# gradslam/gradslam

Measured on AMD Instinct MI355X. Metric: frames/sec PointFusion 640x480 RGB-D, higher is better.
Workload: dtype f32

## Files before the change

gradslam_amd/_C.py:

```python
import ctypes as C
import os

import torch

_HERE = os.path.dirname(os.path.abspath(__file__))
LIB_PATH = os.environ.get("GRADSLAM_HIP_LIB") or os.path.join(_HERE, "csrc", "libgradslam_hip.so")
if os.environ.get("GRADSLAM_HIP_LIB"):
    import warnings
    warnings.warn("GRADSLAM_HIP_LIB overrides the product library: %s" % LIB_PATH, RuntimeWarning)
ABI_VERSION = 3

_lib = None

_vp, _i64, _i32, _f = C.c_void_p, C.c_int64, C.c_int, C.c_float


class IcpParams(C.Structure):
    _fields_ = [("mode", C.c_int), ("numiters", C.c_int), ("damp", C.c_float),
                ("dist_thresh", C.c_float), ("lambda_max", C.c_float), ("B", C.c_float),
                ("B2", C.c_float), ("nu", C.c_float)]


class MapView(C.Structure):
    _fields_ = [("points", C.c_void_p), ("normals", C.c_void_p), ("colors", C.c_void_p), ("ccounts", C.c_void_p),
                ("capacity", C.c_int64), ("n_bound", C.c_int64), ("n_dev", C.c_void_p)]


class LocalizeSeq(C.Structure):
    _fields_ = [("vertex", C.c_void_p), ("depth", C.c_void_p), ("K16", C.c_void_p), ("prev_pose16", C.c_void_p),
                ("map", MapView), ("out_pose16", C.c_void_p), ("scratch", C.c_void_p)]


class UpdateSeq(C.Structure):
    _fields_ = [("map", MapView), ("vertex", C.c_void_p), ("normal", C.c_void_p), ("depth", C.c_void_p),
                ("rgb", C.c_void_p), ("alpha", C.c_void_p), ("pose16", C.c_void_p), ("K16", C.c_void_p),
                ("gvertex", C.c_void_p), ("gnormal", C.c_void_p), ("best_pix", C.c_void_p),
                ("new_count_out", C.c_void_p), ("scratch", C.c_void_p)]


class StepSeq(C.Structure):
    _fields_ = [("depth", C.c_void_p), ("rgb", C.c_void_p), ("K16", C.c_void_p), ("prev_pose16", C.c_void_p),
                ("out_pose16", C.c_void_p), ("vertex", C.c_void_p), ("normal", C.c_void_p), ("alpha", C.c_void_p),
                ("gvertex", C.c_void_p), ("gnormal", C.c_void_p), ("best_pix", C.c_void_p),
                ("new_count_out", C.c_void_p), ("map", MapView), ("loc_scratch", C.c_void_p),
                ("upd_scratch", C.c_void_p)]


class RenderSeq(C.Structure):
    _fields_ = [("map", MapView), ("poses16", C.c_void_p), ("K16", C.c_void_p), ("depth", C.c_void_p),
                ("color", C.c_void_p), ("normal", C.c_void_p), ("confidence", C.c_void_p), ("index", C.c_void_p),
                ("scratch", C.c_void_p)]


class RenderBackwardSeq(C.Structure):
    _fields_ = [("map", MapView), ("poses16", C.c_void_p), ("K16", C.c_void_p), ("index", C.c_void_p),
                ("depth_bar", C.c_void_p), ("color_bar", C.c_void_p), ("normal_bar", C.c_void_p),
                ("confidence_bar", C.c_void_p), ("points_bar", C.c_void_p), ("normals_bar", C.c_void_p),
                ("colors_bar", C.c_void_p), ("ccounts_bar", C.c_void_p), ("poses_bar", C.c_void_p),
                ("scratch", C.c_void_p)]


_PROTOS = {
    "gs_abi_version": [],
    "gs_last_error": [],
    "gs_scratch_bytes": [_i64, _i64],
    "gs_profile_begin": [_i32],
    "gs_profile_end": [],
    "gs_profile_read": [_i32, C.POINTER(C.c_double), C.POINTER(C.c_int64), C.POINTER(C.c_double)],
    "gs_frame_maps_f32": [_vp, _vp, _i32, _i32, _f, _vp, _vp, _vp, _vp, _vp],
    "gs_global_maps_f32": [_vp, _vp, _vp, _vp, _i32, _i32, _vp, _vp, _vp],
    "gs_alpha_f32": [_vp, _i64, _f, _f, _vp, _vp],
    "gs_alpha_backward_f32": [_vp, _i64, _f, _f, _vp, _vp, _vp, _vp],
    "gs_downsample_frame_f32": [_vp, _vp, _vp, _vp, _i32, _i32, _i32, _vp, _vp, _vp, _vp, _vp, _vp],
    "gs_project_map_f32": [_vp, _i64, _vp, _vp, _i32, _i32, _vp, _vp],
    "gs_active_table_i64": [_vp, _i64, _i32, _i64, _vp, _vp, _vp, _vp],
    "gs_select_targets_f32": [_vp, _i64, _i32, _i32, _vp, _vp, _vp, _vp, _vp, _vp, _i64, _vp, _vp, _vp],
    "gs_downsample_table_f32": [_vp, _i64, _i32, _vp, _vp, _vp, _vp, _vp, _vp, _vp, _vp, _vp],
    "gs_knn1_f32": [_vp, _i64, _vp, _i64, _vp, _vp, _vp, _vp],
    "gs_knn1_grid_scratch_bytes": [_i64, _i64],
    "gs_knn1_grid_f32": [_vp, _i64, _vp, _i64, _vp, _vp, _vp, C.POINTER(C.c_int64), _vp],
    "gs_gauss_newton_rows_f32": [_vp, _i64, _vp, _vp, _i64, _f, _vp, _vp, _vp, _vp, _vp, _vp],
    "gs_solve_normal_eq_f32": [_vp, _vp, _vp, _i64, _i32, _f, _vp, _vp],
    "gs_se3_exp_f32": [_vp, _vp, _vp],
    "gs_se3_exp_backward_f32": [_vp, _vp, _vp, _vp],
    "gs_transform_points_f32": [_vp, _i64, _vp, _vp, _vp],
    "gs_icp_scratch_bytes": [_i64, _i64],
    "gs_icp_f32": [_vp, _i64, _vp, _vp, _i64, _vp, _vp, C.POINTER(IcpParams), _vp, _vp, _vp, _vp],
    "gs_icp_trace_f32": [_vp, _i32, _vp, _vp],
    "gs_icp_dc_f32": [_vp, _i64, _vp, _vp, _vp, _i64, _vp, _vp, _vp, C.POINTER(IcpParams), _vp, _vp, _vp, _vp],
    "gs_frame_maps_backward_f32": [_vp, _vp, _i32, _i32, _f, _vp, _vp, _vp, _vp, _vp, _vp, _vp, _vp],
    "gs_frame_maps_backward_kbar_scratch_bytes": [_i32, _i32],
    "gs_global_maps_backward_f32": [_vp, _vp, _vp, _vp, _i32, _i32, _vp, _vp, _vp],
    "gs_downsample_frame_backward_f32": [_vp, _vp, _i32, _i32, _i32, _vp, _vp, _vp],
    "gs_icp_tape_bytes": [_i64, _i32],
    "gs_icp_tape_f32": [_vp, _i64, _vp, _vp, _i64, _vp, _vp, C.POINTER(IcpParams), _vp, _vp, _vp, _vp, _vp],
    "gs_icp_backward_scratch_bytes": [_i64, _i64],
    "gs_icp_backward_f32": [_vp, _vp, _i64, _vp, _vp, _i64, _vp, C.POINTER(IcpParams), _vp, _vp, _vp, _vp, _vp, _vp,
                            _vp],
    "gs_similar_rows_f32": [_vp, _i64, _vp, _vp, _vp, _vp, _i32, _f, _f, _vp, _vp],
    "gs_best_unique_rows_f32": [_vp, _i64, _vp, _vp, _vp, _i32, _i32, _i64, _vp, _vp, _vp, _vp, _vp],
    "gs_associate_f32": [_vp, _i64, _vp, _vp, _vp, _vp, _vp, _i32, _i32, _f, _f, _vp, _vp, _vp, _vp],
    "gs_best_table_i64": [_vp, _i32, _i32, _i64, _vp, _vp, _vp, _vp],
    "gs_rows_to_best_pix": [_vp, _i64, _i32, _i32, _vp, _vp],
    "gs_fuse_append_f32": [_vp, _vp, _vp, _vp, _i64, _i64, _vp, _vp, _vp, _vp, _vp, _vp, _i32, _i32, _i32,
                           _vp, _vp, _vp],
    "gs_append_valid_f32": [_vp, _vp, _vp, _vp, _i64, _i64, _vp, _vp, _vp, _vp, _vp, _i32, _i32, _vp, _vp, _vp],
    "gs_ingest_depth_u16_f32": [_vp, _i32, _i32, _vp, _i32, _i32, C.c_double, _vp],
    "gs_ingest_color_u8_f32": [_vp, _i32, _i32, _vp, _i32, _i32, _i32, _vp],
    "gs_ingest_frames_native_f32": [_vp, _vp, _i64, _i32, _i32, C.c_double, _i32, _vp, _vp, _vp],
    "gs_host_device_pointer": [_vp, C.POINTER(C.c_void_p)],
    "gs_global_maps_pose_backward_scratch_bytes": [_i32, _i32],
    "gs_global_maps_pose_backward_f32": [_vp, _vp, _vp, _vp, _vp, _i32, _i32, _vp, _vp, _vp],
    "gs_fuse_append_backward_f32": [_vp, _vp, _vp, _vp, _i64, _vp, _vp, _vp, _vp, _vp, _vp, _i32, _i32, _i32, _vp, _vp,
                                    _vp, _vp, _i64, _vp, _vp, _vp, _vp, _vp, _vp, _vp, _vp, _vp, _vp],
    "gs_update_map_scratch_bytes": [_i64, _i32, _i32],
    "gs_update_map_fusion_dc_f32": [_vp, _vp, _vp, _vp, _i64, _vp, _i64, _vp, _vp, _vp, _vp, _vp, _vp, _vp, _i32, _i32,
                                    _f, _f, _i32, _vp, _vp, _vp, _vp, _vp, _vp],
    "gs_icp_map_dc_f32": [_vp, _i64, _vp, _vp, _vp, _vp, _i64, _vp, _i32, _i32, _vp, _vp, C.POINTER(IcpParams), _vp, _vp,
                          _vp],
    "gs_lattice_source_f32": [_vp, _vp, _vp, _i32, _i32, _i32, _vp, _vp],
    "gs_relative_pose_f32": [_vp, _vp, _i64, _vp, _vp],
    "gs_project_map_dc_f32": [_vp, _i64, _vp, _vp, _vp, _i32, _i32, _vp, _vp],
    "gs_select_targets_dc_f32": [_vp, _i64, _vp, _i32, _i32, _vp, _vp, _vp, _vp, _vp, _vp, _i64, _vp, _vp, _vp],
    "gs_associate_dc_f32": [_vp, _i64, _vp, _vp, _vp, _vp, _vp, _vp, _i32, _i32, _f, _f, _vp, _vp, _vp, _vp],
    "gs_fuse_append_dc_f32": [_vp, _vp, _vp, _vp, _i64, _vp, _i64, _vp, _vp, _vp, _vp, _vp, _vp, _i32, _i32, _i32,
                              _vp, _vp, _vp],
    "gs_append_valid_dc_f32": [_vp, _vp, _vp, _vp, _i64, _vp, _i64, _vp, _vp, _vp, _vp, _vp, _i32, _i32, _vp, _vp,
                               _vp],
    "gs_frame_maps_batch_f32": [_vp, _i64, _i64, _vp, _i32, _i32, _i32, _i32, _f, _vp, _vp, _vp, _vp],
    "gs_localize_scratch_bytes": [_i32, _i32, _i32, _i64],
    "gs_localize_batch_f32": [C.POINTER(LocalizeSeq), _i32, _i32, _i32, _i32, C.POINTER(IcpParams), _vp],
    "gs_update_map_fusion_batch_f32": [C.POINTER(UpdateSeq), _i32, _i32, _i32, _f, _f, _i32, _vp],
    "gs_project_points_f32": [_vp, _i32, _i64, _vp, _i64, _vp, _vp],
    "gs_unproject_points_f32": [_vp, _i32, _i64, _vp, _i64, _vp, _vp, _vp],
    "gs_lie_small_f32": [_i32, _vp, _vp, _vp],
    "gs_localize_far_stats_i64": [_vp, _i32, _i32, _i32, _i64, C.POINTER(C.c_int64), _vp],
    "gs_localize_list_stats_i64": [_vp, _i32, _i32, _i32, _i64, C.POINTER(C.c_int64), _vp],
    "gs_localize_solve_stats_i64": [_vp, _i32, _i32, _i32, _i64, C.POINTER(C.c_int64), _vp],
    "gs_pointfusion_step_batch_f32": [C.POINTER(StepSeq), _i32, _i32, _i32, _i32, C.POINTER(IcpParams), _f, _f, _f, _i32, _vp],
    "gs_render_scratch_bytes": [_i32, _i32, _i32],
    "gs_render_map_dc_f32": [C.POINTER(RenderSeq), _i32, _i32, _i32, _i32, _i32, _f, _i32, _vp],
    "gs_render_backward_scratch_bytes": [_i32, _i32, _i32, _i64],
    "gs_render_map_backward_dc_f32": [C.POINTER(RenderBackwardSeq), _i32, _i32, _i32, _i32, _i32, _vp],
}
_RESTYPE = {"gs_last_error": C.c_char_p, "gs_scratch_bytes": _i64, "gs_icp_scratch_bytes": _i64,
            "gs_knn1_grid_scratch_bytes": _i64, "gs_update_map_scratch_bytes": _i64, "gs_global_maps_pose_backward_scratch_bytes": _i64, "gs_icp_tape_bytes": _i64, "gs_icp_backward_scratch_bytes": _i64,
            "gs_localize_scratch_bytes": _i64, "gs_frame_maps_backward_kbar_scratch_bytes": _i64,
            "gs_render_scratch_bytes": _i64, "gs_render_backward_scratch_bytes": _i64}
EXPORTS = tuple(_PROTOS)


class HipExtensionError(RuntimeError):
    pass


def lib():
    global _lib
    if _lib is None:
        if not os.path.exists(LIB_PATH):
            raise HipExtensionError(
                "gradslam_amd: %s is missing. Build it with `python -m gradslam_amd.csrc.build` "
                "(hipcc --offload-arch=gfx950). There is no CPU / PyTorch fallback." % LIB_PATH)
        handle = C.CDLL(LIB_PATH)
        for name, argtypes in _PROTOS.items():
            fn = getattr(handle, name)
            fn.argtypes = argtypes
            fn.restype = _RESTYPE.get(name, C.c_int)
        if handle.gs_abi_version() != ABI_VERSION:
            raise HipExtensionError("libgradslam_hip.so ABI %d != expected %d; rebuild"
                                    % (handle.gs_abi_version(), ABI_VERSION))
        _lib = handle
    return _lib


def check(status, what):
    if status != 0:
        raise HipExtensionError("%s failed (code %d): %s" % (what, status, lib().gs_last_error().decode()))


def require_device(*tensors):
    dev = None
    for t in tensors:
        if t is None:
            continue
        if not t.is_cuda:
            raise HipExtensionError(
                "gradslam_amd kernels run on the GPU only (got a %s tensor). Move the data to a HIP "
                "device; there is no CPU fallback." % t.device)
        if not t.is_contiguous():
            raise HipExtensionError("internal error: non-contiguous tensor passed to the HIP library")
        if dev is None:
            dev = t.device
        elif t.device != dev:
            raise HipExtensionError("tensors live on different devices: %s vs %s" % (dev, t.device))
    return dev


def ptr(t):
    return None if t is None else C.c_void_p(t.data_ptr())


def stream(device):
    return C.c_void_p(torch.cuda.current_stream(device).cuda_stream)


class Workspace:
    _instances = {}

    def __init__(self, device):
        self.device = device
        self._bufs = {}

    @classmethod
    def get(cls, device):
        device = torch.device(device)
        if device.index is None:
            device = torch.device("cuda", torch.cuda.current_device())
        key = (device, torch.cuda.current_stream(device).cuda_stream)
        ws = cls._instances.get(key)
        if ws is None:
            ws = cls._instances[key] = Workspace(device)
        return ws

    def bytes(self, name, nbytes):
        buf = self._bufs.get(name)
        if buf is None or buf.numel() < nbytes:
            nbytes = int(nbytes * 1.5) + 4096
            buf = self._bufs[name] = torch.empty(nbytes, dtype=torch.uint8, device=self.device)
        return buf

    def scratch(self, n_map, n_pix):
        return self.bytes("scratch", lib().gs_scratch_bytes(int(n_map), int(n_pix)))

    def tensor(self, name, shape, dtype):
        n = 1
        for s in shape:
            n *= int(s)
        item = torch.empty((), dtype=dtype).element_size()
        buf = self.bytes(name, max(n, 1) * item)
        return buf[: n * item].view(dtype).view(*shape)
```

gradslam_amd/csrc/gs_icp_loop.hip:

```cpp
#include <stdlib.h>
#include <string.h>

#include <memory>
#include <mutex>
#include <type_traits>

#include "gs_env.h"
#include "gs_icp_math.h"
#include "gs_knn.h"
#include "gs_knn_bbox.h"

constexpr int GS_ICP_MAX_ITERS = 1024;
struct GsIcpState {
  IcpSmall s[2];
  float trace[GS_ICP_MAX_ITERS * 12];
};

struct TapePtrs {
  float* src;
  int32_t* idx;
  float* sys;
};
GS_DEV void tape_write_sys(float* __restrict__ sys, int it, const double* S, float damp) {
  float* t = sys + 28 * it;
// ... 1127 lines not shown
  float* lattice;
  GsIcpState* state;
  float* out_pose16;
  char* clear_ptr;
  int64_t* n_valid;
  int* far_n;
  int* lstat;
  float4* wl_cq;
  unsigned* sync;
};
struct LocBatch {
  int B, W, ds, Wl;
  int64_t n_lat;
  size_t clear_bytes;
  float damp;
  int numiters;
  int count_valid;
  LocSeq s[GS_MAX_BATCH];
};
constexpr int LP_CLEAR_ITEMS = 8;

GS_DEV void loc_prep_block(const LocBatch& lb, const unsigned bid, const unsigned nb_lat) {
  const LocSeq& q = lb.s[bid % lb.B];
  const unsigned blk = bid / lb.B;
  if (blk < nb_lat) {
    const int64_t e = (int64_t)blk * 256 + threadIdx.x;
    int valid = 0;
    if (e < lb.n_lat) {
      const int64_t p = (e / lb.Wl) * lb.ds * (int64_t)lb.W + (e % lb.Wl) * lb.ds;
      float g0 = __builtin_nanf(""), g1 = g0, g2 = g0;
      if (q.depth[p] > 0.0f) {
        float T[12];
#pragma unroll
        for (int i = 0; i < 12; ++i) T[i] = q.pose16[i];
        gs_rigid_fma(T, q.vertex[3 * p], q.vertex[3 * p + 1], q.vertex[3 * p + 2], g0, g1, g2);
        valid = 1;
      }
      q.lattice[3 * e] = g0; q.lattice[3 * e + 1] = g1; q.lattice[3 * e + 2] = g2;
      if (q.wl_cq) q.wl_cq[e] = make_float4(0.0f, 0.0f, 0.0f, 0.0f);
    }
    const unsigned long long m = lb.count_valid ? __ballot(valid) : 0ull;
    if ((threadIdx.x & 63) == 0 && m) atomicAdd(reinterpret_cast<unsigned long long*>(q.n_valid), (unsigned long long)__popcll(m));
    if (blk == 0 && threadIdx.x == 0) {
      IcpSmall sm;
      for (int i = 0; i < 16; ++i) {
        const float id = (i % 5 == 0) ? 1.0f : 0.0f;
        sm.T_total[i] = id; sm.T_step[i] = id; sm.Tr[i] = id;
      }
      for (int i = 0; i < 8; ++i) sm.xi[i] = 0.0f;
      sm.damp = lb.damp;
      sm.err = 0.0f;
      sm.pad[0] = sm.pad[1] = 0.0f;
      q.state->s[0] = sm;
      q.state->s[1] = sm;
      if (q.far_n)
        for (int i = 0; i < FS_FAR_PASSES; ++i) q.far_n[i] = 0;
      if (q.lstat)
        for (int i = 0; i < 3 * GL_STAT_LAUNCHES; ++i) q.lstat[i] = 0;
      if (q.sync)
        for (int i = 0; i < PS_WORDS; ++i) q.sync[i] = 0u;
      if (lb.numiters == 0) icp_write_result(sm, q.pose16, q.out_pose16);
    }
    return;
  }
  float4* dst = reinterpret_cast<float4*>(q.clear_ptr);
  const size_t n16 = lb.clear_bytes / 16;
  const size_t base = (size_t)(blk - nb_lat) * 256 * LP_CLEAR_ITEMS + threadIdx.x;
#pragma unroll
  for (int u = 0; u < LP_CLEAR_ITEMS; ++u) {
    const size_t i = base + (size_t)u * 256;
    if (i < n16) dst[i] = make_float4(0.0f, 0.0f, 0.0f, 0.0f);
  }
}
__global__ void __launch_bounds__(256) gs_loc_prep_kernel(const LocBatch lb, unsigned nb_lat) {
  loc_prep_block(lb, blockIdx.x, nb_lat);
}
static_assert(GB_BLOCK == 256, "lattice and bbox blocks share a launch");
__global__ void __launch_bounds__(256) gs_loc_prep_bbox_kernel(const LocBatch lb, const GsGridBatch gb, const unsigned nb_lat,
                                                               const float u_hi, const float v_hi) {
  const unsigned n_prep = (unsigned)lb.B * nb_lat;
  if (blockIdx.x < n_prep) loc_prep_block(lb, blockIdx.x, nb_lat);
  else gridb_bbox_block(gb, blockIdx.x - n_prep, u_hi, v_hi);
}

struct IcpRowsBatch {
  int B;
  const double* in[GS_MAX_BATCH];
  double* out[GS_MAX_BATCH];
};
__global__ void __launch_bounds__(FS_BLOCK) gs_icp_reduce_rows_batch_kernel(const IcpRowsBatch rb, GsCount n_src_c) {
  __shared__ double S[32];
  __shared__ double sub[FS_BLOCK / 32][32];
  const int nrows = (int)((gs_count(n_src_c) + FS_QPB - 1) / FS_QPB);
  icp_sum_rows<FS_BLOCK>(rb.in[blockIdx.x], nrows, S, sub);
  if (threadIdx.x < LIN_NV) rb.out[blockIdx.x][threadIdx.x] = S[threadIdx.x];
}

struct IcpFinishBatch {
  int B;
  const double* partials_in[GS_MAX_BATCH];
  GsIcpState* st[GS_MAX_BATCH];
  const float* compose16[GS_MAX_BATCH];
  float* out_T16[GS_MAX_BATCH];
  unsigned* sync[GS_MAX_BATCH];
  int nb, h0;
};
__global__ void __launch_bounds__(FS_BLOCK) gs_icp_finish_batch_kernel(const IcpFinishBatch fb, GsCount n_src_c, int buf,
                                                                       gs_icp_params prm) {
  __shared__ double red[FS_BLOCK / GS_WAVE];
  const int b = blockIdx.x;
  const int nrows_in = (int)((gs_count(n_src_c) + FS_QPB - 1) / FS_QPB);
  const double e1 = icp_sum_col27<FS_BLOCK>(fb.partials_in[b], nrows_in, red);
  if (threadIdx.x != 0) return;
  GsIcpState* st = fb.st[b];
  IcpSmall sm = st->s[buf];
  const int it = prm.numiters - 1;
  icp_update_math((float)e1, sm, prm, it < GS_ICP_MAX_ITERS ? st->trace + 12 * it : nullptr);
  st->s[buf ^ 1] = sm;
  icp_write_result(sm, fb.compose16[b], fb.out_T16[b]);
  if (unsigned* sy = fb.sync[b]) {
    const unsigned arrived = sy[PS_ARRIVED], want = (unsigned)fb.nb * (unsigned)(2 * prm.numiters - fb.h0);
    if (!(sy[PS_ERROR] == 0u && arrived == want && sy[PS_TICKET] >= (unsigned)fb.nb))
      for (int i = 0; i < 16; ++i) fb.out_T16[b][i] = __builtin_nanf("");
    sy[PS_NB] = (unsigned)fb.nb;
    sy[PS_H0] = (unsigned)fb.h0;
  }
}

static int64_t loc_lattice(int H, int W, int ds) { return (int64_t)((H + ds - 1) / ds) * ((W + ds - 1) / ds); }

struct ListMem {
  float4* lq;
  uint32_t* ls;
  int* stat;
};

struct FarMem {
  uint32_t* c;
  float4* cq;
  int* idx;
  int* n;
};

struct FarBuildSeq {
  const float* src;
  const int* idx;
  const int* n;
  const GsGrid* gp;
  const int* cell_start;
  const float4* sorted;
  float* d2prev;
  FarMem m;
};
struct FarBuildBatch {
  int B;
  FarBuildSeq s[GS_MAX_BATCH];
};
constexpr int FAR_BLOCK = 512;
constexpr int FAR_BLOCKS_PER_SEQ = 64;
__global__ void __launch_bounds__(FAR_BLOCK) gs_icp_far_build_kernel(const FarBuildBatch fb) {
  const FarBuildSeq& q = fb.s[blockIdx.x % fb.B];
  const int blk = (int)(blockIdx.x / fb.B);
  const int n = *q.n;
  if (blk >= n) return;
  constexpr int NG = FAR_BLOCK / FS_HG;
  __shared__ float qs[NG][3];
  __shared__ float d1_s[NG];
  __shared__ uint8_t flag_s[NG];
  __shared__ int unres_q[NG], sq_s[NG];
  __shared__ int unres_n;
  __shared__ uint32_t stage_s[NG][GS_FAR_SLOTS + 4];
  const GsGrid g = *q.gp;
  const int grp = threadIdx.x / FS_HG, l16 = threadIdx.x & (FS_HG - 1);
  for (int base = blk; base < n; base += FAR_BLOCKS_PER_SEQ * NG) {
    if (threadIdx.x == 0) unres_n = 0;
    __syncthreads();
    const int e = base + grp * FAR_BLOCKS_PER_SEQ;
    if (e < n) {
      const int sq = q.idx[e];
      const float hx = q.src[3 * (int64_t)sq], hy = q.src[3 * (int64_t)sq + 1], hz = q.src[3 * (int64_t)sq + 2];
      const float4 found = q.m.cq[sq];
      const float d1 = sqrtf(found.x);
      const int kdone = (int)found.y;
      if (kdone >= 0) {
        const float R = far_emit_cube<FS_HG>(g, q.cell_start, q.sorted, hx, hy, hz, l16, d1, kdone, stage_s[grp],
                                             reinterpret_cast<int*>(&stage_s[grp][GS_FAR_SLOTS]));
        for (int u = l16; u < GS_FAR_SLOTS; u += FS_HG) q.m.c[GS_FAR_SLOTS * (int64_t)sq + u] = stage_s[grp][u];
        if (l16 == 0) {
          q.m.cq[sq] = make_float4(hx, hy, hz, R);
          if (R > 0.0f) q.d2prev[sq] = __uint_as_float(__float_as_uint(q.d2prev[sq]) | 0x80000000u);
        }
      } else if (l16 == 0) {
        qs[grp][0] = hx; qs[grp][1] = hy; qs[grp][2] = hz;
        d1_s[grp] = d1;
        sq_s[grp] = sq;
        unres_q[atomicAdd(&unres_n, 1)] = grp;
      }
    }
    __syncthreads();
    const int nun = unres_n;
    for (int u = 0; u < nun; u += FS_BQ) {
      const int nq = nun - u < FS_BQ ? nun - u : FS_BQ;
      block_brute_collect_multi<FAR_BLOCK, FS_BQ>(qs, unres_q + u, nq, q.sorted, q.cell_start[g.ncell], d1_s,
                                                  GS_FAR_RADD * g.c, sq_s, q.m.cq, q.m.c, flag_s);
      if ((int)threadIdx.x < nq) {
        const int gq = unres_q[u + threadIdx.x];
        const int s2 = sq_s[gq];
        if (flag_s[gq]) q.d2prev[s2] = __uint_as_float(__float_as_uint(q.d2prev[s2]) | 0x80000000u);
      }
    }
    __syncthreads();
  }
}

static int64_t loc_rows(const gs_map_view& m) { return m.capacity > m.n_bound ? m.capacity : m.n_bound; }

struct LocLayout {
  int64_t n_lat, rows;
  IcpLayout sc;
  size_t lattice, pix, n_valid, icp, lq, ls, lstat, far_c, far_cq, far_idx, far_n, far_out4, total;
};
static LocLayout loc_layout(int64_t n_lat, int64_t rows) {
  GsTake take;
  LocLayout L;
  L.n_lat = n_lat; L.rows = rows > 0 ? rows : 1;
  L.lattice = take(gs_align(12 * (size_t)n_lat));
  L.pix = take(gs_align(4 * (size_t)L.rows));
  L.n_valid = take(256);
  L.sc = icp_layout(n_lat, L.rows);
  L.icp = take(L.sc.total);
  L.lq = take(gs_align(16 * (size_t)n_lat));
  L.ls = take(gs_align(4 * GL_SLOTS * (size_t)n_lat));
  L.lstat = take(gs_align(4 * 3 * GL_STAT_LAUNCHES));
  L.far_c = take(gs_align(4 * GS_FAR_SLOTS * (size_t)n_lat));
  L.far_cq = take(gs_align(16 * (size_t)n_lat));
  L.far_idx = take(gs_align(4 * FS_FAR_PASSES * (size_t)n_lat));
  L.far_n = take(256);
  L.far_out4 = L.far_n + 4 * 8;
  static_assert(FS_FAR_PASSES <= 8, "the far-list counters run into the result words");
  L.total = take.end;
  return L;
}
static bool loc_lists_fit(const LocLayout& L) { return L.total - (L.icp + L.sc.partials[1]) >= sizeof(double) * LIN_NV * FS_BLOCK; }

extern "C" int64_t gs_localize_scratch_bytes(int H, int W, int ds, int64_t n_map_bound) {
  if (H < 1 || W < 1 || ds < 1) return 0;
  return (int64_t)loc_layout(loc_lattice(H, W, ds), n_map_bound).total;
}

struct LocCarve {
  float* lattice; int32_t* pix; int64_t* n_valid;
  IcpScratch sc; GridMem gm; ListMem lm;
  FarMem fm; int* far_out4;
};
static LocCarve loc_carve(void* p, const LocLayout& L) {
  const IcpScratch sc = icp_carve(gs_at<char>(p, L.icp), L.sc);
  return LocCarve{gs_at<float>(p, L.lattice), gs_at<int32_t>(p, L.pix), gs_at<int64_t>(p, L.n_valid), sc,
                  grid_carve(sc.grid, L.n_lat, L.rows),
                  ListMem{gs_at<float4>(p, L.lq), gs_at<uint32_t>(p, L.ls), gs_at<int>(p, L.lstat)},
                  FarMem{gs_at<uint32_t>(p, L.far_c), gs_at<float4>(p, L.far_cq), gs_at<int>(p, L.far_idx), gs_at<int>(p, L.far_n)},
                  gs_at<int>(p, L.far_out4)};
}
static LocCarve loc_carve_of(const void* scratch, int H, int W, int ds, int64_t map_rows) {
  return loc_carve(const_cast<void*>(scratch), loc_layout(loc_lattice(H, W, ds), map_rows));
}

struct IcpEnginePlan {
  bool far_on, wide_on, lists_on, persist_on;
  bool binned_normals;
  bool reduce_rows;
  int lists_from;
  IcpHalfPlan half;
  int ps_it0, ps_nb, ps_upb;
  float weak_room;
  int lmode(int it, bool look_ahead) const {
    if (!lists_on || it < lists_from) return 0;
    if (it > lists_from) return 2;
    return look_ahead ? (persist_on ? 3 : 1) : 0;
  }
};
static IcpEnginePlan icp_engine_plan(const GsEnv& env, const IcpDevice& dev, int B, int64_t n_lat, int numiters,
                                     const LocLayout* layouts) {
  IcpEnginePlan p;
  const int64_t rows = (int64_t)icp_rows(n_lat);
  p.binned_normals = env.icp_binned_normals; p.weak_room = env.icp_weak_room;
  p.lists_from = env.icp_lists_from >= 0 ? env.icp_lists_from : FS_LISTS_FROM;
  p.reduce_rows = rows > FS_REDUCE_ROWS;
  p.far_on = env.icp_far && numiters > 0;
  p.wide_on = env.icp_wide && !p.far_on && numiters > 0;
  p.ps_upb = (int)gs_ceil_div(rows, PS_CUS_PER_XCD);
  p.ps_nb = (int)gs_ceil_div(rows, p.ps_upb > 0 ? p.ps_upb : 1);
  const bool persist_asked = env.icp_persist && env.icp_lists && !p.far_on && B <= (int)GS_XCDS && p.ps_upb <= PS_UPB &&
                             numiters > p.lists_from + 1 && !env.icp_timeline && !env.icp_lanes_set && dev.ps_fits &&
                             p.binned_normals;
  p.half = icp_half_plan(env, dev.cus, n_lat, B, p.far_on ? 4 : (persist_asked ? 2 : 8));
  p.lists_on = env.icp_lists && !p.far_on && p.half.upb * p.half.G * FS_QPB <= FS_BLOCK;
  for (int b = 0; b < B && p.lists_on; ++b) p.lists_on = loc_lists_fit(layouts[b]);
  p.persist_on = persist_asked && p.half.G == 2 && p.lists_on;
  p.ps_it0 = p.persist_on ? p.lists_from + 1 : numiters;
  return p;
}

static void loc_bind(const gs_localize_seq* seqs, int B, int H, int W, int ds, const gs_icp_params* prm,
                     const IcpEnginePlan& plan, LocCarve* c, LocBatch& lb, GsGridBatch& gb) {
  lb.B = gb.B = B; lb.W = gb.W = W; gb.H = H; lb.ds = gb.ds = ds;
  lb.Wl = (W + ds - 1) / ds; lb.n_lat = loc_lattice(H, W, ds); lb.damp = prm->damp; lb.numiters = prm->numiters;
  gb.cells_cap = gs_knn_grid_cells_cap(lb.n_lat);
  for (int b = 0; b < B; ++b) {
    const gs_localize_seq& q = seqs[b];
    if (!plan.binned_normals) c[b].gm.sorted_n = nullptr;
    lb.s[b] = LocSeq{q.vertex, q.depth, q.prev_pose16, c[b].lattice, c[b].sc.state, q.out_pose16,
                     reinterpret_cast<char*>(c[b].gm.g), c[b].n_valid, c[b].fm.n, c[b].lm.stat,
                     plan.wide_on ? c[b].fm.cq : nullptr, c[b].sc.sync};
    gb.s[b] = GsGridSeq{q.map.points, GsCount{q.map.n_bound, q.map.n_dev}, c[b].pix, q.prev_pose16, q.K16,
                        plan.binned_normals ? q.map.normals : nullptr, c[b].gm};
  }
  lb.count_valid = g_gs_prof_on ? 1 : 0;
  lb.clear_bytes = gs_knn_grid_clear_bytes(c[0].gm, gb.cells_cap);
}

static int loc_prep(const gs_localize_seq* seqs, const LocBatch& lb, const GsGridBatch& gb, hipStream_t st, bool grid_cleared) {
  const int B = lb.B;
  if (g_gs_prof_on)
    for (int b = 0; b < B; ++b) GS_HIP(hipMemsetAsync(lb.s[b].n_valid, 0, 8, st));
  const unsigned nb_lat = (unsigned)gs_ceil_div(lb.n_lat, 256);
  const unsigned nb_clear = (unsigned)gs_ceil_div((int64_t)(lb.clear_bytes / 16), 256 * LP_CLEAR_ITEMS);
  double bytes = 0.0;
  for (int b = 0; b < B; ++b) bytes += 28.0 * lb.n_lat + 24.0 * seqs[b].map.n_bound + 16.0 * gb.cells_cap;
  GsProf prof(GS_PROF_COMPACT, bytes, st, grid_cleared ? 4 : 5);
  if (grid_cleared) {
    const float u_hi = (float)((double)gb.W - 0.999), v_hi = (float)((double)gb.H - 0.999);
    hipLaunchKernelGGL(gs_loc_prep_bbox_kernel, dim3((unsigned)B * nb_lat + gs_knn_gridb_bbox_blocks(gb)), dim3(256), 0, st,
                       lb, gb, nb_lat, u_hi, v_hi);
    return gs_knn_grid_build_batch(gb, st, true);
  }
  hipLaunchKernelGGL(gs_loc_prep_kernel, dim3((unsigned)B * (nb_lat + nb_clear)), dim3(256), 0, st, lb, nb_lat);
  return gs_knn_grid_build_batch(gb, st);
}

static int loc_prof_bytes(int B, const LocCarve* c, int64_t n_lat, int numiters, hipStream_t st, double* bytes) {
  for (int b = 0; b < B; ++b) {
    unsigned hits = 0; int64_t nv = 0;
    GS_HIP(hipMemcpyAsync(&hits, c[b].gm.bbox + 6, 4, hipMemcpyDeviceToHost, st));
    GS_HIP(hipMemcpyAsync(&nv, c[b].n_valid, 8, hipMemcpyDeviceToHost, st));
    GS_HIP(hipStreamSynchronize(st));
    *bytes += icp_alg_bytes(numiters, n_lat, nv, hits);
  }
  return GS_OK;
}

static void loc_half_iterations(const gs_localize_seq* seqs, int B, const IcpEnginePlan& plan, const LocCarve* c,
                                int64_t n_lat, const gs_icp_params* prm, hipStream_t st) {
  const GsCount n_src_c{n_lat, nullptr};
  const FarMem no_far{nullptr, nullptr, nullptr, nullptr};
  IcpHalfBatch hb;
  hb.B = B; hb.weak_room = plan.weak_room;
  for (int it = 0; it < plan.ps_it0; ++it) {
    int h = 2 * it;
    for (int b = 0; b < B; ++b) {
      const gs_localize_seq& q = seqs[b];
      const IcpScratch& sc = c[b].sc; const GridMem& gm = c[b].gm;
      const FarMem& fm = plan.far_on ? c[b].fm : no_far;
      const float* cur_in = it == 0 ? c[b].lattice : (((it - 1) & 1) ? sc.srcB : sc.srcA);
      float* cur = (it & 1) ? sc.srcB : sc.srcA;
      hb.s[b] = IcpHalfSeq{cur_in, cur, q.map.points, q.map.normals, GsCount{q.map.n_bound, q.map.n_dev}, gm.g,
                           gm.cell_start, gm.sorted, gm.sorted_n, reinterpret_cast<float*>(sc.best),
                           sc.partials[(h + 1) & 1], sc.partials[h & 1], &sc.state->s[h & 1], &sc.state->s[(h + 1) & 1],
                           sc.state->trace, nullptr, nullptr, nullptr, fm.cq, fm.c, fm.idx, fm.n};
      hb.w[b] = plan.wide_on ? IcpHalfWide{c[b].fm.cq, c[b].fm.c} : IcpHalfWide{nullptr, nullptr};
      hb.l[b] = plan.lists_on ? IcpHalfLists{c[b].lm.lq, c[b].lm.ls, c[b].lm.stat, sc.sync + PS_WEAK}
                              : IcpHalfLists{nullptr, nullptr, nullptr, nullptr};
    }
    icp_half_launch<true>(plan.half, hb, n_src_c, prm, it, 0, st, plan.lmode(it, false));
    if (plan.far_on && fs_far_pass(it) >= 0) {
      const int fp = fs_far_pass(it);
      FarBuildBatch fbb; fbb.B = B;
      for (int b = 0; b < B; ++b)
        fbb.s[b] = FarBuildSeq{(it & 1) ? c[b].sc.srcB : c[b].sc.srcA, c[b].fm.idx + (int64_t)fp * n_lat, c[b].fm.n + fp,
                               c[b].gm.g, c[b].gm.cell_start, c[b].gm.sorted, reinterpret_cast<float*>(c[b].sc.best), c[b].fm};
      hipLaunchKernelGGL(gs_icp_far_build_kernel, dim3((unsigned)B * FAR_BLOCKS_PER_SEQ), dim3(FAR_BLOCK), 0, st, fbb);
    }
    ++h;
    if (plan.reduce_rows) {
      IcpRowsBatch rb; rb.B = B;
      for (int b = 0; b < B; ++b) { rb.in[b] = c[b].sc.partials[(h + 1) & 1]; rb.out[b] = c[b].sc.rowred; }
      hipLaunchKernelGGL(gs_icp_reduce_rows_batch_kernel, dim3((unsigned)B), dim3(FS_BLOCK), 0, st, rb, n_src_c);
    }
    for (int b = 0; b < B; ++b) {
      const IcpScratch& sc = c[b].sc;
      IcpHalfSeq& u = hb.s[b];
      u.src_in = (it & 1) ? sc.srcB : sc.srcA; u.src_out = nullptr;
      u.partials_in = plan.reduce_rows ? sc.rowred : sc.partials[(h + 1) & 1];
      u.partials_out = sc.partials[h & 1];
      u.st_in = &sc.state->s[h & 1]; u.st_out = &sc.state->s[(h + 1) & 1];
    }
    icp_half_launch<false>(plan.half, hb, n_src_c, prm, it, plan.reduce_rows ? 1 : 0, st, plan.lmode(it, true));
  }
}

static void loc_persist(const gs_localize_seq* seqs, int B, const IcpEnginePlan& plan, const LocCarve* c, int64_t n_lat,
                        const gs_icp_params* prm, hipStream_t st) {
  IcpPersistBatch pb;
  pb.B = B; pb.nb = plan.ps_nb; pb.upb = plan.ps_upb; pb.h0 = 2 * plan.ps_it0; pb.tl_h = 0; pb.timeline = nullptr;
  for (int b = 0; b < B; ++b) {
    const gs_localize_seq& q = seqs[b];
    const IcpScratch& sc = c[b].sc; const GridMem& gm = c[b].gm;
    pb.s[b] = IcpPersistSeq{((plan.ps_it0 - 1) & 1) ? sc.srcB : sc.srcA, GsCount{q.map.n_bound, q.map.n_dev}, gm.g, gm.cell_start,
                            gm.sorted, gm.sorted_n, {sc.partials[0], sc.partials[1]}, sc.state, c[b].lm.lq, c[b].lm.ls,
                            c[b].lm.stat, plan.wide_on ? c[b].fm.cq : nullptr, plan.wide_on ? c[b].fm.c : nullptr, sc.sync};
  }
#ifdef GS_ICP_TIMELINE
  ps_tl_arm(pb, prm->numiters, st);
#endif
  hipLaunchKernelGGL(gs_icp_persist_kernel, dim3(GS_XCDS * PS_CUS_PER_XCD), dim3(PS_BLOCK), 0, st, pb, n_lat, prm->dist_thresh, *prm);
#ifdef GS_ICP_TIMELINE
  ps_tl_dump(pb, st);
#endif
}

static void loc_finish(const gs_localize_seq* seqs, int B, const IcpEnginePlan& plan, const LocCarve* c, int64_t n_lat,
                       const gs_icp_params* prm, hipStream_t st) {
  const int h = 2 * prm->numiters;
  GsProf prof(GS_PROF_SOLVE, 1.0, st);
  IcpFinishBatch fb;
  fb.B = B; fb.nb = plan.persist_on ? plan.ps_nb : 0; fb.h0 = plan.persist_on ? 2 * plan.ps_it0 : 0;
  for (int b = 0; b < B; ++b) {
    fb.partials_in[b] = c[b].sc.partials[(h + 1) & 1];
    fb.st[b] = c[b].sc.state; fb.compose16[b] = seqs[b].prev_pose16; fb.out_T16[b] = seqs[b].out_pose16;
    fb.sync[b] = plan.persist_on ? c[b].sc.sync : nullptr;
  }
  hipLaunchKernelGGL(gs_icp_finish_batch_kernel, dim3((unsigned)B), dim3(FS_BLOCK), 0, st, fb, GsCount{n_lat, nullptr}, h & 1, *prm);
}

static int localize_chunk(const gs_localize_seq* seqs, int B, int H, int W, int ds, const gs_icp_params* prm,
                          hipStream_t st, bool grid_cleared) {
  const int64_t n_lat = loc_lattice(H, W, ds);
  LocLayout layouts[GS_MAX_BATCH]; LocCarve c[GS_MAX_BATCH];
  for (int b = 0; b < B; ++b) {
    layouts[b] = loc_layout(n_lat, loc_rows(seqs[b].map));
    c[b] = loc_carve(seqs[b].scratch, layouts[b]);
  }
  const IcpEnginePlan plan = icp_engine_plan(gs_env(), icp_device(), B, n_lat, prm->numiters, layouts);
  LocBatch lb; GsGridBatch gb;
  loc_bind(seqs, B, H, W, ds, prm, plan, c, lb, gb);
  int rc = loc_prep(seqs, lb, gb, st, grid_cleared);
  if (rc != GS_OK) return rc;
  if (prm->numiters == 0) { GS_LAUNCH_CHECK(); return GS_OK; }
  double prof_bytes = 0.0;
  if (g_gs_prof_on && (rc = loc_prof_bytes(B, c, n_lat, prm->numiters, st, &prof_bytes)) != GS_OK) return rc;
  {
    GsProf prof(GS_PROF_ICP_FUSED, prof_bytes, st, 2 * prm->numiters);
    loc_half_iterations(seqs, B, plan, c, n_lat, prm, st);
    if (plan.persist_on) loc_persist(seqs, B, plan, c, n_lat, prm, st);
  }
  loc_finish(seqs, B, plan, c, n_lat, prm, st);
  GS_LAUNCH_CHECK();
  return GS_OK;
}

static int localize_batch(const gs_localize_seq* seqs_host, int B, int H, int W, int ds, const gs_icp_params* prm,
                          void* stream, bool grid_cleared) {
  GS_REQUIRE(seqs_host && prm && B > 0 && H > 0 && W > 0 && ds > 0, "bad arguments");
  GS_REQUIRE(prm->numiters >= 0 && prm->numiters <= GS_ICP_MAX_ITERS, "numiters must be in [0, 1024]");
  GS_REQUIRE(prm->mode == 0 || prm->mode == 1, "mode must be 0 (ICP) or 1 (gradICP)");
  GS_REQUIRE((int64_t)H * W < (1ll << 31), "image too large for int32 pixel ids");
  for (int b = 0; b < B; ++b) {
    const gs_localize_seq& q = seqs_host[b];
    GS_REQUIRE(q.vertex && q.depth && q.K16 && q.prev_pose16 && q.out_pose16 && q.scratch, "NULL pointer");
    GS_REQUIRE(q.map.points && q.map.normals && q.map.n_bound > 0 && q.map.n_bound < 0x7fffffffll,
               "every sequence needs a non-empty map (points + normals)");
    GS_REQUIRE(q.map.capacity <= 0 || q.map.n_bound <= q.map.capacity, "map.n_bound exceeds map.capacity");
  }
  hipStream_t st = gs_stream(stream);
  for (int c0 = 0; c0 < B; c0 += GS_MAX_BATCH) {
    const int nb = B - c0 < GS_MAX_BATCH ? B - c0 : GS_MAX_BATCH;
    const int rc = localize_chunk(seqs_host + c0, nb, H, W, ds, prm, st, grid_cleared);
    if (rc != GS_OK) return rc;
  }
  return GS_OK;
}
extern "C" int gs_localize_batch_f32(const gs_localize_seq* seqs_host, int B, int H, int W, int ds,
                                     const gs_icp_params* prm, void* stream) {
  return localize_batch(seqs_host, B, H, W, ds, prm, stream, false);
}

__global__ void __launch_bounds__(256) gs_far_stats_kernel(const int* __restrict__ far_idx, const int* __restrict__ far_n,
                                                          const float* __restrict__ d2prev, const float4* __restrict__ far_cq,
                                                          int64_t n_lat, int* __restrict__ out4) {
  const int n0 = far_n[0], n = n0 < 0 ? 0 : (n0 > (int)n_lat ? (int)n_lat : n0);
  if (blockIdx.x == 0 && threadIdx.x == 0) { out4[0] = n; out4[2] = far_n[1]; }
  int c = 0, built = 0;
  for (int i = blockIdx.x * 256 + threadIdx.x; i < n; i += gridDim.x * 256) {
    const int s = far_idx[i];
    if (s < 0 || s >= (int)n_lat) continue;
    c += (__float_as_uint(d2prev[s]) >> 31) ? 1 : 0;
    built += far_cq[s].w > 0.0f ? 1 : 0;
  }
  if (c) atomicAdd(&out4[1], c);
  if (built) atomicAdd(&out4[3], built);
}
extern "C" int gs_localize_far_stats_i64(const void* scratch, int H, int W, int ds, int64_t map_rows, int64_t* out4_host,
                                         void* stream) {
  GS_REQUIRE(scratch && out4_host && H > 0 && W > 0 && ds > 0 && map_rows > 0, "bad arguments");
  const int64_t n_lat = loc_lattice(H, W, ds);
  const LocCarve cv = loc_carve_of(scratch, H, W, ds, map_rows);
  const FarMem& fm = cv.fm; hipStream_t st = gs_stream(stream);
  int* out4 = cv.far_out4;
  GS_HIP(hipMemsetAsync(out4, 0, 16, st));
  hipLaunchKernelGGL(gs_far_stats_kernel, dim3(64), dim3(256), 0, st, fm.idx, fm.n, reinterpret_cast<const float*>(cv.sc.best),
                     fm.cq, n_lat, out4);
  int h[4] = {0, 0, 0, 0};
  GsGrid g;
  GS_HIP(hipMemcpyAsync(h, out4, 16, hipMemcpyDeviceToHost, st));
  GS_HIP(hipMemcpyAsync(&g, cv.gm.g, sizeof(g), hipMemcpyDeviceToHost, st));
  GS_HIP(hipStreamSynchronize(st));
  for (int i = 0; i < 4; ++i) out4_host[i] = h[i];
  if (gs_env().debug_grid)
    fprintf(stderr, "grid: box (%.3f %.3f %.3f)-(%.3f %.3f %.3f) c %.4f cells %d x %d x %d = %d\n", g.ox, g.oy, g.oz, g.mx,
            g.my, g.mz, g.c, g.nx, g.ny, g.nz, g.ncell);
  return GS_OK;
}

extern "C" int gs_localize_list_stats_i64(const void* scratch, int H, int W, int ds, int64_t map_rows, int64_t* out192_host,
                                          void* stream) {
  GS_REQUIRE(scratch && out192_host && H > 0 && W > 0 && ds > 0 && map_rows > 0, "bad arguments");
  const ListMem lm = loc_carve_of(scratch, H, W, ds, map_rows).lm;
  int h[3 * GL_STAT_LAUNCHES];
  hipStream_t st = gs_stream(stream);
  GS_HIP(hipMemcpyAsync(h, lm.stat, sizeof(h), hipMemcpyDeviceToHost, st));
  GS_HIP(hipStreamSynchronize(st));
  for (int i = 0; i < 3 * GL_STAT_LAUNCHES; ++i) out192_host[i] = h[i];
  return GS_OK;
}

extern "C" int gs_localize_solve_stats_i64(const void* scratch, int H, int W, int ds, int64_t map_rows, int64_t* out8_host,
                                           void* stream) {
  GS_REQUIRE(scratch && out8_host && H > 0 && W > 0 && ds > 0 && map_rows > 0, "bad arguments");
  const LocCarve cv = loc_carve_of(scratch, H, W, ds, map_rows);
  unsigned h[PS_WORDS];
  hipStream_t st = gs_stream(stream);
  GS_HIP(hipMemcpyAsync(h, cv.sc.sync, sizeof(h), hipMemcpyDeviceToHost, st));
  GS_HIP(hipStreamSynchronize(st));
  static_assert(PS_WORDS == 8, "out8");
  for (int i = 0; i < PS_WORDS; ++i) out8_host[i] = h[i];
  return GS_OK;
}

extern "C" int gs_pointfusion_step_batch_f32(const gs_step_seq* seqs_host, int B, int H, int W, int ds,
                                             const gs_icp_params* prm, float two_sigma_sq, float dist_th, float dot_th,
                                             int renorm_all, void* stream) {
  GS_REQUIRE(seqs_host && prm && B > 0 && H > 0 && W > 0 && ds > 0, "bad arguments");
  const int64_t P = (int64_t)H * W;
  const gs_step_seq& s0 = seqs_host[0];
  const int64_t dstride = B > 1 ? seqs_host[1].depth - s0.depth : P;
  for (int b = 0; b < B; ++b) {
    const gs_step_seq& q = seqs_host[b];
    GS_REQUIRE(q.depth && q.rgb && q.K16 && q.prev_pose16 && q.out_pose16 && q.vertex && q.normal && q.alpha &&
                   q.best_pix && q.new_count_out && q.loc_scratch && q.upd_scratch, "NULL pointer");
    GS_REQUIRE((q.gvertex != nullptr) == (q.gnormal != nullptr) && (q.gvertex != nullptr) == (s0.gvertex != nullptr),
               "gvertex / gnormal: both or none, the same choice for every sequence");
    GS_REQUIRE(q.out_pose16 != q.prev_pose16, "out_pose16 must not alias prev_pose16");
    GS_REQUIRE(q.vertex == s0.vertex + 3 * P * b && q.normal == s0.normal + 3 * P * b && q.alpha == s0.alpha + P * b,
               "vertex / normal / alpha of the batch must be dense");
    GS_REQUIRE(q.depth == s0.depth + dstride * b && q.K16 == s0.K16 + 16 * (int64_t)b, "depth / K16 must be equally strided");
  }
  GS_REQUIRE(dstride >= P || B == 1, "overlapping depth images");
  const bool implicit_global = s0.gvertex == nullptr;
  std::unique_ptr<gs_update_seq[]> us(new gs_update_seq[B]);
  for (int c0 = 0; c0 < B; c0 += GS_MAX_BATCH) {
    const int nb = B - c0 < GS_MAX_BATCH ? B - c0 : GS_MAX_BATCH;
    const gs_step_seq* sq = seqs_host + c0;
    gs_localize_seq ls[GS_MAX_BATCH];
    for (int b = 0; b < nb; ++b) {
      const gs_step_seq& q = sq[b];
      ls[b].vertex = q.vertex; ls[b].depth = q.depth; ls[b].K16 = q.K16; ls[b].prev_pose16 = q.prev_pose16;
      ls[b].map = q.map; ls[b].out_pose16 = q.out_pose16; ls[b].scratch = q.loc_scratch;
      gs_update_seq& u = us[c0 + b];
      u.map = q.map; u.vertex = q.vertex; u.normal = q.normal; u.depth = q.depth; u.rgb = q.rgb;
      u.alpha = q.alpha; u.pose16 = q.out_pose16; u.K16 = q.K16; u.gvertex = q.gvertex;
      u.gnormal = q.gnormal; u.best_pix = q.best_pix; u.new_count_out = q.new_count_out;
      u.scratch = q.upd_scratch;
    }
    GsClearJob job;
    job.n = nb;
    for (int b = 0; b < nb; ++b) {
      GS_REQUIRE(ls[b].map.points && ls[b].map.n_bound > 0, "every sequence needs a non-empty map");
      const LocCarve cv = loc_carve_of(ls[b].scratch, H, W, ds, loc_rows(ls[b].map));
      job.ptr[b] = reinterpret_cast<char*>(cv.gm.g);
      if (b == 0) job.bytes = gs_knn_grid_clear_bytes(cv.gm, gs_knn_grid_cells_cap(loc_lattice(H, W, ds)));
    }
    GsPixelTables tabs{};
    tabs.n = implicit_global ? nb : 0;
    tabs.call_flag = c0 == 0 ? gs_update_map_call_flag(seqs_host[0].upd_scratch) : nullptr;
    for (int b = 0; b < tabs.n; ++b) {
      gs_update_map_tables(sq[b].upd_scratch, &tabs.any_flag[b], &tabs.key_pix[b]);
      tabs.best_pix[b] = sq[b].best_pix;
    }
    int rc = gs_frame_maps_batch_clear(sq[0].depth, dstride, P, sq[0].K16, nb, 1, H, W, two_sigma_sq, sq[0].vertex,
                                       sq[0].normal, sq[0].alpha, &job, stream, &tabs);
    if (rc != GS_OK) return rc;
    rc = localize_batch(ls, nb, H, W, ds, prm, stream, true);
    if (rc != GS_OK) return rc;
  }
  return gs_update_map_fusion_batch_impl(us.get(), B, H, W, dist_th, dot_th, renorm_all, stream, implicit_global);
}

extern "C" int64_t gs_icp_tape_bytes(int64_t n_src, int numiters) { return (int64_t)gs_icp_tape_size(n_src, numiters); }

extern "C" int gs_icp_tape_f32(const float* src, int64_t n_src, const float* tgt, const float* tgt_normals,
                               int64_t n_tgt, const float* init16, const float* compose16,
                               const gs_icp_params* prm, float* out_T16, int64_t* out_idx, void* icp_scratch,
                               void* tape, void* stream) {
  GS_REQUIRE(tape, "tape must not be NULL");
  return icp_run(src, n_src, tgt, tgt_normals, n_tgt, init16, compose16, prm, out_T16, out_idx, icp_scratch, tape,
                 stream);
}

extern "C" int gs_icp_trace_f32(const void* icp_scratch, int numiters, float* trace_out, void* stream) {
  GS_REQUIRE(icp_scratch && trace_out && numiters >= 0 && numiters <= GS_ICP_MAX_ITERS, "bad arguments");
  const GsIcpState* st = reinterpret_cast<const GsIcpState*>(icp_scratch);
  GS_HIP(hipMemcpyAsync(trace_out, st->trace, sizeof(float) * 12 * (size_t)numiters, hipMemcpyDeviceToDevice,
                        gs_stream(stream)));
  return GS_OK;
}
```

gradslam_amd/csrc/gs_knn.h:

```cpp
#pragma once
#include "gs_common.h"

GS_DEV unsigned long long knn_pack(float d, uint32_t idx) {
  return ((unsigned long long)__float_as_uint(d) << 32) | (unsigned long long)idx;
}

int gs_knn_brute_launch(const float* src_in, const float* Tapply, float* src_out, int64_t n_src,
                        const float* tgt, int64_t n_tgt, unsigned long long* best, hipStream_t st);

constexpr int GS_GRID_MAXCELL = 1 << 22;
constexpr int GS_GRID_RINGS = 3;
constexpr int GS_GRID_TILE = 1024;

struct GsGrid {
  float ox, oy, oz;
  float mx, my, mz;
  float c, inv_c;
  int nx, ny, nz, ncell;
};

struct GsTargetFilter {
  const int32_t* pix;
  int W, ds;
};
GS_DEV bool gs_is_target(const GsTargetFilter& f, int64_t n) {
  if (!f.pix) return true;
  const int32_t p = f.pix[n];
  return p >= 0 && ((p / f.W) % f.ds == 0) && ((p % f.W) % f.ds == 0);
}

struct GridMem {
  GsGrid* g;
  unsigned* bbox;
  int* unres_count;
  int* cell_count;
  int* cell_start;
  int* tile_sums;
  float4* sorted;
  float4* sorted_n;
  float4* tlist;
  int* unres_list;
};

static inline GridMem grid_carve(void* scratch, int64_t n_src, int64_t n_tgt) {
  char* p = reinterpret_cast<char*>(scratch);
  GridMem m;
  m.g = reinterpret_cast<GsGrid*>(p); p += 128;
  m.bbox = reinterpret_cast<unsigned*>(p); p += 128;
  m.unres_count = reinterpret_cast<int*>(p); p += 256;
  m.tile_sums = reinterpret_cast<int*>(p); p += gs_align(4 * (size_t)(GS_GRID_MAXCELL / GS_GRID_TILE + 2));
  m.cell_count = reinterpret_cast<int*>(p); p += gs_align(4 * (size_t)(GS_GRID_MAXCELL + 1));
  m.cell_start = reinterpret_cast<int*>(p); p += gs_align(4 * (size_t)(GS_GRID_MAXCELL + 1));
  m.sorted = reinterpret_cast<float4*>(p); p += gs_align(16 * (size_t)(n_tgt > 0 ? n_tgt : 1));
  m.sorted_n = reinterpret_cast<float4*>(p); p += gs_align(16 * (size_t)(n_tgt > 0 ? n_tgt : 1));
  m.tlist = reinterpret_cast<float4*>(p); p += gs_align(16 * (size_t)(n_tgt > 0 ? n_tgt : 1));
  m.unres_list = reinterpret_cast<int*>(p);
  (void)n_src;
  return m;
}

size_t gs_knn_grid_scratch_bytes(int64_t n_src, int64_t n_tgt);

struct GsGridSeq {
  const float* tgt;
  GsCount n_tgt;
  int32_t* pix;
  const float* pose16;
  const float* K16;
  const float* nrm;
  GridMem m;
};
struct GsGridBatch {
  int B, H, W, ds;
  int cells_cap;
  GsGridSeq s[GS_MAX_BATCH];
};
int gs_knn_grid_cells_cap(int64_t n_src);
size_t gs_knn_grid_clear_bytes(const GridMem& m, int cells_cap);
int gs_knn_grid_build_batch(const GsGridBatch& gb, hipStream_t st, bool bbox_done = false);

int gs_knn_grid_build(const float* tgt, GsCount n_tgt, int64_t n_src, void* grid_scratch, hipStream_t st,
                      GsTargetFilter filter = GsTargetFilter{nullptr, 1, 1}, const float* nrm = nullptr);
int gs_knn_grid_query(const float* src_in, const float* Tapply, float* src_out, int64_t n_src,
                      const float* tgt, int64_t n_tgt, unsigned long long* best, void* grid_scratch,
                      hipStream_t st);
static inline bool gs_knn_use_grid(int64_t n_src, int64_t n_tgt) { return n_tgt >= 2048 && n_src >= 256; }

GS_DEV int grid_axis(float v, float o, float inv_c, int n) {
  const float f = (v - o) * inv_c;
  return f >= 0.0f ? (f < (float)n ? (int)f : n - 1) : 0;
}
GS_DEV int grid_cell(const GsGrid& g, float x, float y, float z) {
  const int ix = grid_axis(x, g.ox, g.inv_c, g.nx);
  const int iy = grid_axis(y, g.oy, g.inv_c, g.ny);
  const int iz = grid_axis(z, g.oz, g.inv_c, g.nz);
  return (iz * g.ny + iy) * g.nx + ix;
}

constexpr int GQ_G = 8;
constexpr int GL_RING_NF = 2;

GS_DEV unsigned long long grid_key(float qx, float qy, float qz, const float4 p) {
  const float dx = qx - p.x, dy = qy - p.y, dz = qz - p.z;
  float d = dx * dx;
  d = gs_fma(dy, dy, d);
  d = gs_fma(dz, dz, d);
  return d == d ? knn_pack(d, (uint32_t)__float_as_int(p.w)) : ~0ull;
}

template <int G>
GS_DEV unsigned long long grid_group_min(unsigned long long key) {
#pragma unroll
  for (int d = G / 2; d > 0; d >>= 1) {
    const unsigned long long o = __shfl_xor(key, d, G);
    key = o < key ? o : key;
  }
  return key;
}

struct GsQueryCell {
  float px, py, pz;
  int cx, cy, cz;
};
GS_DEV GsQueryCell grid_query_cell(const GsGrid& g, float qx, float qy, float qz) {
  GsQueryCell c;
  c.px = qx < g.ox ? g.ox : (qx > g.mx ? g.mx : qx);
  c.py = qy < g.oy ? g.oy : (qy > g.my ? g.my : qy);
  c.pz = qz < g.oz ? g.oz : (qz > g.mz ? g.mz : qz);
  c.cx = grid_axis(c.px, g.ox, g.inv_c, g.nx); c.cy = grid_axis(c.py, g.oy, g.inv_c, g.ny);
  c.cz = grid_axis(c.pz, g.oz, g.inv_c, g.nz);
  return c;
}

template <int G>
GS_DEV unsigned long long grid_search_stage0(const GsGrid& g, const int* __restrict__ cell_start,
                                             const float4* __restrict__ sorted, float qx, float qy, float qz, int lane,
                                             bool* resolved, int* win, const float rball = __builtin_inff()) {
  const GsQueryCell qc = grid_query_cell(g, qx, qy, qz);
  const float px = qc.px, py = qc.py, pz = qc.pz;
  const int cx = qc.cx, cy = qc.cy, cz = qc.cz;
  unsigned long long key = ~0ull;
  int bt = -1;
  const float fx = (px - g.ox) * g.inv_c - (float)cx, fy = (py - g.oy) * g.inv_c - (float)cy,
              fz = (pz - g.oz) * g.inv_c - (float)cz;
  const int x0 = (fx < 0.5f) ? cx - 1 : cx, y0 = (fy < 0.5f) ? cy - 1 : cy, z0 = (fz < 0.5f) ? cz - 1 : cz;
  const float BIG = 3.0e38f;
  const float ax = fminf(x0 >= 1 ? fx + (float)(cx - x0) : BIG, x0 + 2 < g.nx ? (float)(x0 + 2 - cx) - fx : BIG);
  const float ay = fminf(y0 >= 1 ? fy + (float)(cy - y0) : BIG, y0 + 2 < g.ny ? (float)(y0 + 2 - cy) - fy : BIG);
  const float az = fminf(z0 >= 1 ? fz + (float)(cz - z0) : BIG, z0 + 2 < g.nz ? (float)(z0 + 2 - cz) - fz : BIG);
  const float amin = fminf(ax, fminf(ay, az));
  const float rc = rball * g.inv_c * 1.0001f + 0.002f;
  const bool prune = rc < amin - 0.001f;
  bool ulx = true, uhx = true, uly = true, uhy = true, ulz = true, uhz = true;
  if (prune) {
    const float tx = fx + (float)(cx - x0), ty = fy + (float)(cy - y0), tz = fz + (float)(cz - z0);
    ulx = tx - rc < 1.0f; uhx = tx + rc >= 1.0f;
    uly = ty - rc < 1.0f; uhy = ty + rc >= 1.0f;
    ulz = tz - rc < 1.0f; uhz = tz + rc >= 1.0f;
  }
  int sb0 = 0, sb1 = 0, sb2 = 0, sb3 = 0, e1 = 0, e2 = 0, e3 = 0, total = 0;
  {
    const int xa = (x0 >= 0 && ulx) ? x0 : x0 + 1, xb = (x0 + 1 < g.nx && uhx) ? x0 + 1 : x0;
    const bool zl = z0 >= 0 && ulz, zh = z0 + 1 < g.nz && uhz, yl = y0 >= 0 && uly, yh = y0 + 1 < g.ny && uhy;
    const int r0 = (z0 * g.ny + y0) * g.nx, r1 = r0 + g.nx, r2 = r0 + g.ny * g.nx, r3 = r2 + g.nx;
    int se0 = 0, se1 = 0, se2 = 0, se3 = 0;
    if (zl && yl) { sb0 = cell_start[r0 + xa]; se0 = cell_start[r0 + xb + 1]; }
    if (zl && yh) { sb1 = cell_start[r1 + xa]; se1 = cell_start[r1 + xb + 1]; }
    if (zh && yl) { sb2 = cell_start[r2 + xa]; se2 = cell_start[r2 + xb + 1]; }
    if (zh && yh) { sb3 = cell_start[r3 + xa]; se3 = cell_start[r3 + xb + 1]; }
    e1 = se0 - sb0;
    e2 = e1 + (se1 - sb1);
    e3 = e2 + (se2 - sb2);
    total = e3 + (se3 - sb3);
  }
  for (int t0 = lane; t0 < total; t0 += 4 * G) {
    float4 p[4];
    bool in[4];
#pragma unroll
    for (int u = 0; u < 4; ++u) {
      const int t = t0 + u * G;
      in[u] = t < total;
      const int tt = in[u] ? t : 0;
      const int ix = tt < e1 ? sb0 + tt : (tt < e2 ? sb1 + (tt - e1) : (tt < e3 ? sb2 + (tt - e2) : sb3 + (tt - e3)));
      p[u] = sorted[ix];
    }
#pragma unroll
    for (int u = 0; u < 4; ++u) {
      const unsigned long long k2 = in[u] ? grid_key(qx, qy, qz, p[u]) : ~0ull;
      const bool better = k2 < key;
      key = better ? k2 : key;
      bt = better ? t0 + u * G : bt;
    }
  }
  {
    const unsigned long long kmin = grid_group_min<G>(key);
    const int bs = bt < e1 ? sb0 + bt : (bt < e2 ? sb1 + (bt - e1) : (bt < e3 ? sb2 + (bt - e2) : sb3 + (bt - e3)));
    *win = (key == kmin && bt >= 0) ? bs : -1;
    key = kmin;
  }
  const float rb = (amin < 1.0e30f) ? (amin - 0.001f) * g.c : BIG;
  const float bd = __uint_as_float((uint32_t)(key >> 32));
  *resolved = prune ? (bd == bd) : (rb > 0.0f && (rb >= 1.0e30f ? bd == bd : bd <= rb * rb));
  return key;
}

template <int G>
GS_DEV unsigned long long grid_search_rings(const GsGrid& g, const int* __restrict__ cell_start,
                                            const float4* __restrict__ sorted, float qx, float qy, float qz, int lane,
                                            unsigned long long key, bool* resolved, int* win,
                                            const int kmax = GS_GRID_RINGS, int* kdone = nullptr) {
  const GsQueryCell qc = grid_query_cell(g, qx, qy, qz);
  bool done = false;
  int bs = -1;
  int k = 1;
  for (; k <= kmax && !done; ++k) {
    const int side = 2 * k + 1, nrow = side * side;
    const int xa = qc.cx - k < 0 ? 0 : qc.cx - k, xb = qc.cx + k >= g.nx ? g.nx - 1 : qc.cx + k;
    for (int r = lane; r < nrow; r += G) {
      const int zz = qc.cz + r / side - k, yy = qc.cy + r % side - k;
      if (zz < 0 || zz >= g.nz || yy < 0 || yy >= g.ny) continue;
      const int row = (zz * g.ny + yy) * g.nx;
      const int je = cell_start[row + xb + 1];
      for (int j = cell_start[row + xa]; j < je; j += GL_RING_NF) {
        float4 p[GL_RING_NF];
#pragma unroll
        for (int u = 0; u < GL_RING_NF; ++u) p[u] = sorted[j + u < je ? j + u : je - 1];
#pragma unroll
        for (int u = 0; u < GL_RING_NF; ++u) {
          const unsigned long long k2 = j + u < je ? grid_key(qx, qy, qz, p[u]) : ~0ull;
          if (k2 < key) { key = k2; bs = j + u; }
        }
      }
    }
    {
      const unsigned long long own = key;
      key = grid_group_min<G>(key);
      if (own != key) bs = -1;
    }
    const float rb = (float)k * g.c * 0.999f;
    const float bd = __uint_as_float((uint32_t)(key >> 32));
    done = bd <= rb * rb;
  }
  *resolved = done;
  *win = bs;
  if (kdone) *kdone = k - 1;
  return key;
}

constexpr int GS_FAR_SLOTS = 64;
constexpr float GS_FAR_RADD = 1.0f;

template <int G>
GS_DEV unsigned long long far_list_search(const float4 c0R, const uint32_t* __restrict__ slots,
                                          const float4* __restrict__ sorted, float qx, float qy, float qz, int lane,
                                          bool* proven, int* win) {
  static_assert(GS_FAR_SLOTS == 4 * G, "four list entries per lane");
  const uint4 sl = reinterpret_cast<const uint4*>(slots)[lane];
  const uint32_t s4[4] = {sl.x, sl.y, sl.z, sl.w};
  float4 a[4];
#pragma unroll
  for (int u = 0; u < 4; ++u) a[u] = sorted[s4[u] != ~0u ? s4[u] : 0u];
  unsigned long long k = ~0ull;
  int bs = -1;
#pragma unroll
  for (int u = 0; u < 4; ++u) {
    const unsigned long long k2 = s4[u] != ~0u ? grid_key(qx, qy, qz, a[u]) : ~0ull;
    if (k2 < k) { k = k2; bs = (int)s4[u]; }
  }
  const unsigned long long kmin = grid_group_min<G>(k);
  *win = (k == kmin) ? bs : -1;
  const float bd = __uint_as_float((uint32_t)(kmin >> 32));
  const float ex = qx - c0R.x, ey = qy - c0R.y, ez = qz - c0R.z;
  const float delta = sqrtf(ex * ex + ey * ey + ez * ez);
  *proven = sqrtf(bd) + delta < c0R.w * 0.9999f;
  return kmin;
}

template <int G>
GS_DEV unsigned long long wide_list_search(const float4 c0R, const uint32_t* __restrict__ slots,
                                           const float4* __restrict__ sorted, float qx, float qy, float qz, int lane,
                                           bool* proven, int* win) {
  static_assert(GS_FAR_SLOTS == 4 * G, "four list entries per lane");
  unsigned long long k = ~0ull;
  int bs = -1;
#pragma unroll
  for (int h = 0; h < 2; ++h) {
    const uint2 sl = reinterpret_cast<const uint2*>(slots)[2 * lane + h];
    const float4 a0 = sorted[sl.x != ~0u ? sl.x : 0u], a1 = sorted[sl.y != ~0u ? sl.y : 0u];
    const unsigned long long k0 = sl.x != ~0u ? grid_key(qx, qy, qz, a0) : ~0ull;
    const unsigned long long k1 = sl.y != ~0u ? grid_key(qx, qy, qz, a1) : ~0ull;
    if (k0 < k) { k = k0; bs = (int)sl.x; }
    if (k1 < k) { k = k1; bs = (int)sl.y; }
  }
  const unsigned long long kmin = grid_group_min<G>(k);
  *win = (k == kmin) ? bs : -1;
  const float bd = __uint_as_float((uint32_t)(kmin >> 32));
  const float ex = qx - c0R.x, ey = qy - c0R.y, ez = qz - c0R.z;
  const float delta = sqrtf(ex * ex + ey * ey + ez * ez);
  *proven = sqrtf(bd) + delta < c0R.w * 0.9999f;
  return kmin;
}

template <int G>
GS_DEV float far_emit_cube(const GsGrid& g, const int* __restrict__ cell_start, const float4* __restrict__ sorted,
                           float qx, float qy, float qz, int lane, const float d1, const int kdone, uint32_t* stage,
                           int* stage_n) {
  const GsQueryCell qc = grid_query_cell(g, qx, qy, qz);
  float radd = GS_FAR_RADD * g.c, R = 0.0f;
  const int kE = (d1 + radd > (float)kdone * g.c * 0.999f) ? kdone + 1 : kdone;
  const int xa = qc.cx - kE < 0 ? 0 : qc.cx - kE, xb = qc.cx + kE >= g.nx ? g.nx - 1 : qc.cx + kE;
  const int side = 2 * kE + 1, nrow = side * side;
  const float rcube = (float)kE * g.c * 0.999f;
  for (int attempt = 0; attempt < 3; ++attempt, radd *= 0.5f) {
    float Rt = d1 + radd;
    Rt = Rt < rcube ? Rt : rcube;
    const float R2 = Rt * Rt;
    if (lane == 0) *stage_n = 0;
    for (int u = lane; u < GS_FAR_SLOTS; u += G) stage[u] = ~0u;
    __builtin_amdgcn_fence(__ATOMIC_RELEASE, "wavefront");
    __builtin_amdgcn_wave_barrier();
    for (int r = lane; r < nrow; r += G) {
      const int zz = qc.cz + r / side - kE, yy = qc.cy + r % side - kE;
      if (zz < 0 || zz >= g.nz || yy < 0 || yy >= g.ny) continue;
      const int row = (zz * g.ny + yy) * g.nx;
      const int je = cell_start[row + xb + 1];
      for (int j = cell_start[row + xa]; j < je; ++j) {
        const float4 c = sorted[j];
        const float dx = qx - c.x, dy = qy - c.y, dz = qz - c.z;
        float d = dx * dx;
        d = gs_fma(dy, dy, d);
        d = gs_fma(dz, dz, d);
        if (d < R2) {
          const int pos = atomicAdd(stage_n, 1);
          if (pos < GS_FAR_SLOTS) stage[pos] = (uint32_t)j;
        }
      }
    }
    __builtin_amdgcn_fence(__ATOMIC_ACQ_REL, "wavefront");
    __builtin_amdgcn_wave_barrier();
    const int n = *stage_n;
    __builtin_amdgcn_wave_barrier();
    if (n <= GS_FAR_SLOTS) { R = Rt; break; }
  }
  return R;
}

constexpr int GL_SLOTS = 8;
constexpr int GL_STAT_LAUNCHES = 64;
constexpr float GL_MIN_ROOM = 0.1f;
template <int G> constexpr int gl_k() { return G == 2 ? 2 : 1; }

template <int KT>
struct GlTop {
  float d[KT + 1];
  int s[KT];
};
template <int KT>
GS_DEV void gl_top_reset(GlTop<KT>& t) {
#pragma unroll
  for (int k = 0; k <= KT; ++k) t.d[k] = __builtin_inff();
#pragma unroll
  for (int k = 0; k < KT; ++k) t.s[k] = -1;
}
template <int KT>
GS_DEV void gl_top_push(GlTop<KT>& t, const float d, const int slot) {
#pragma unroll
  for (int k = KT; k >= 0; --k) {
    const bool before_prev = k > 0 && d < t.d[k - 1];
    const bool before_this = d < t.d[k];
    if (k < KT) t.s[k] = before_prev ? t.s[k - 1] : (before_this ? slot : t.s[k]);
    t.d[k] = before_prev ? t.d[k - 1] : (before_this ? d : t.d[k]);
  }
}
template <int G>
GS_DEV float gl_group_minf(float v) {
#pragma unroll
  for (int d = G / 2; d > 0; d >>= 1) {
    const float o = __shfl_xor(v, d, G);
    v = o < v ? o : v;
  }
  return v;
}

template <int G, int KT, int NFI = (G >= 16 ? 1 : 4)>
GS_DEV unsigned long long grid_search_stage0_top(const GsGrid& g, const int* __restrict__ cell_start,
// ... 400 lines not shown
```

gradslam_amd/csrc/gs_knn.hip:

```cpp
#include "gs_knn.h"

#include <stdlib.h>

#include "gs_assoc_dev.h"
#include "gs_env.h"
#include "gs_knn_bbox.h"

constexpr int KNN_BLOCK = 256;
constexpr int KNN_TCHUNK = 512;

template <bool LISTED, int KNN_SPT>
__global__ void __launch_bounds__(KNN_BLOCK) gs_knn1_kernel(
    const float* __restrict__ src_in, const float* __restrict__ Tapply, float* __restrict__ src_out,
    int64_t n_src, const float* __restrict__ tgt, int64_t n_tgt, unsigned long long* __restrict__ best,
    const int* __restrict__ list, const int* __restrict__ count) {
  constexpr int KNN_STILE = KNN_BLOCK * KNN_SPT;
  __shared__ float4 tl[KNN_TCHUNK];
  const int64_t n_q = LISTED ? (int64_t)(*count) : n_src;
  if (LISTED && n_q == 0) return;
  const int64_t j0 = (int64_t)blockIdx.y * KNN_TCHUNK;
  const int cnt = (int)((n_tgt - j0) < KNN_TCHUNK ? (n_tgt - j0) : KNN_TCHUNK);
  if (cnt <= 0) return;
  for (int i = threadIdx.x; i < cnt; i += KNN_BLOCK) {
    const float* t = tgt + 3 * (j0 + i);
    tl[i] = make_float4(t[0], t[1], t[2], 0.0f);
  }
  float T[12];
  if (Tapply) {
#pragma unroll
    for (int i = 0; i < 12; ++i) T[i] = Tapply[i];
  }
  __syncthreads();
  for (int64_t tile = blockIdx.x; tile * KNN_STILE < n_q; tile += gridDim.x) {
    float sx[KNN_SPT], sy[KNN_SPT], sz[KNN_SPT], bd[KNN_SPT];
    int bi[KNN_SPT];
    int64_t sidx[KNN_SPT];
#pragma unroll
    for (int k = 0; k < KNN_SPT; ++k) {
      const int64_t q = tile * KNN_STILE + k * KNN_BLOCK + threadIdx.x;
      int64_t s = -1;
      if (q < n_q) s = LISTED ? (int64_t)list[q] : q;
      float p0 = 0.0f, p1 = 0.0f, p2 = 0.0f;
      if (s >= 0) {
        p0 = src_in[3 * s];
        p1 = src_in[3 * s + 1];
        p2 = src_in[3 * s + 2];
        if (Tapply) {
          float q0, q1, q2;
          gs_rigid_fma(T, p0, p1, p2, q0, q1, q2);
          p0 = q0; p1 = q1; p2 = q2;
        }
        if (!LISTED && src_out && blockIdx.y == 0) {
          src_out[3 * s] = p0;
          src_out[3 * s + 1] = p1;
          src_out[3 * s + 2] = p2;
        }
      }
      sidx[k] = s;
      sx[k] = p0; sy[k] = p1; sz[k] = p2;
      bd[k] = __builtin_inff();
      bi[k] = 0;
    }
#pragma unroll 4
    for (int j = 0; j < cnt; ++j) {
      const float4 t = tl[j];
#pragma unroll
      for (int k = 0; k < KNN_SPT; ++k) {
        const float dx = sx[k] - t.x, dy = sy[k] - t.y, dz = sz[k] - t.z;
        float d = dx * dx;
        d = gs_fma(dy, dy, d);
        d = gs_fma(dz, dz, d);
        const bool lt = d < bd[k];
        bd[k] = lt ? d : bd[k];
        bi[k] = lt ? j : bi[k];
      }
    }
#pragma unroll
    for (int k = 0; k < KNN_SPT; ++k)
      if (sidx[k] >= 0) atomicMin(&best[sidx[k]], knn_pack(bd[k], (uint32_t)(j0 + bi[k])));
    if (!LISTED) break;
  }
}

int gs_knn_brute_launch(const float* src_in, const float* Tapply, float* src_out, int64_t n_src,
                        const float* tgt, int64_t n_tgt, unsigned long long* best, hipStream_t st) {
  const int spt_env = gs_env().knn_spt;
  const int spt = spt_env == 4 || spt_env == 8 ? spt_env : (n_src * n_tgt >= (int64_t)1 << 27 ? 8 : 4);
  GsProf prof(GS_PROF_KNN, (double)n_src * (double)n_tgt, st);
  if (spt == 8) {
    dim3 grid((unsigned)gs_ceil_div(n_src, KNN_BLOCK * 8), (unsigned)gs_ceil_div(n_tgt, KNN_TCHUNK));
    hipLaunchKernelGGL((gs_knn1_kernel<false, 8>), grid, dim3(KNN_BLOCK), 0, st, src_in, Tapply, src_out, n_src, tgt,
                       n_tgt, best, nullptr, nullptr);
  } else {
    dim3 grid((unsigned)gs_ceil_div(n_src, KNN_BLOCK * 4), (unsigned)gs_ceil_div(n_tgt, KNN_TCHUNK));
    hipLaunchKernelGGL((gs_knn1_kernel<false, 4>), grid, dim3(KNN_BLOCK), 0, st, src_in, Tapply, src_out, n_src, tgt,
                       n_tgt, best, nullptr, nullptr);
  }
  return GS_OK;
}

size_t gs_knn_grid_scratch_bytes(int64_t n_src, int64_t n_tgt) {
  return 512 + 2 * gs_align(4 * (size_t)(GS_GRID_MAXCELL + 1)) + gs_align(4 * (size_t)(GS_GRID_MAXCELL / GS_GRID_TILE + 2)) +
         3 * gs_align(16 * (size_t)(n_tgt > 0 ? n_tgt : 1)) + gs_align(4 * (size_t)(n_src > 0 ? n_src : 1)) + 256;
}

__global__ void __launch_bounds__(GB_BLOCK) gs_grid_bbox_kernel(const float* __restrict__ tgt, GsCount n_tgt_c,
                                                                 const GsTargetFilter flt,
                                                                 unsigned* __restrict__ bbox,
                                                                 int* __restrict__ unres_count,
                                                                 float4* __restrict__ tlist) {
  grid_bbox_body(tgt, gs_count(n_tgt_c), flt, nullptr, 0, 0.0f, 0.0f, nullptr, bbox, unres_count, tlist, blockIdx.x);
}

GS_DEV GsGrid grid_from_bbox(const unsigned* __restrict__ bbox, int64_t n_tgt, int cells_cap) {
  float o[3], m[3];
#pragma unroll
  for (int k = 0; k < 3; ++k) {
    const unsigned cl = bbox[k], ch = bbox[3 + k];
    float a = 0.0f, b = 0.0f;
    if (cl != 0u && ch != 0u) { a = grid_decode(~cl); b = grid_decode(ch); }
    o[k] = a; m[k] = b;
  }
  const float tiny = 1e-6f;
  const float ex = (m[0] - o[0]) + tiny, ey = (m[1] - o[1]) + tiny, ez = (m[2] - o[2]) + tiny;
  const float n = (float)(n_tgt > 0 ? n_tgt : 1);
  const float area = ex * ey + ey * ez + ex * ez;
  float c = 1.5f * sqrtf(area / n);
  const float cv = 0.5f * cbrtf((ex * ey * ez) / n);
  c = cv > c ? cv : c;
  const float emax = ex > ey ? (ex > ez ? ex : ez) : (ey > ez ? ey : ez);
  c = c > emax * (1.0f / 1024.0f) ? c : emax * (1.0f / 1024.0f);
  c = c > 1e-6f ? c : 1e-6f;
  int nx, ny, nz;
  for (;;) {
    nx = (int)(ex / c) + 1; ny = (int)(ey / c) + 1; nz = (int)(ez / c) + 1;
    if ((double)nx * (double)ny * (double)nz <= (double)cells_cap) break;
    c *= 1.26f;
  }
  GsGrid g;
  g.ox = o[0]; g.oy = o[1]; g.oz = o[2];
  g.mx = m[0]; g.my = m[1]; g.mz = m[2];
  g.c = c; g.inv_c = 1.0f / c;
  g.nx = nx; g.ny = ny; g.nz = nz; g.ncell = nx * ny * nz;
  return g;
}

GS_DEV void grid_count_body(const float* __restrict__ tgt, const int64_t n_tgt, const GsTargetFilter flt,
                            const unsigned* __restrict__ bbox, GsGrid* __restrict__ gp, int* __restrict__ cell_count,
                            int* __restrict__ tile_sums, int cells_cap, const float4* __restrict__ tlist,
                            const unsigned blk, const unsigned nblk) {
  __shared__ GsGrid gsh;
  __shared__ int th[GS_GRID_MAXCELL / GS_GRID_TILE + 1];
  const int64_t n_items = flt.pix ? (int64_t)bbox[6] : n_tgt;
  if ((int64_t)blk * 256 >= n_items && blk != 0) return;
  if (threadIdx.x == 0) {
    gsh = grid_from_bbox(bbox, n_items, cells_cap);
    if (blk == 0) *gp = gsh;
  }
  __syncthreads();
  const GsGrid g = gsh;
  const int ntile = g.ncell / GS_GRID_TILE + 1;
  for (int t = threadIdx.x; t < ntile; t += 256) th[t] = 0;
  __syncthreads();
  if (flt.pix) {
    for (int64_t i = (int64_t)blk * 256 + threadIdx.x; i < n_items; i += (int64_t)nblk * 256) {
      const float4 t = tlist[i];
      const int cid = grid_cell(g, t.x, t.y, t.z);
      atomicAdd(&cell_count[cid], 1);
      atomicAdd(&th[cid / GS_GRID_TILE], 1);
    }
  } else {
    const int64_t i = (int64_t)blk * 256 + threadIdx.x;
    if (i < n_tgt) {
      const int cid = grid_cell(g, tgt[3 * i], tgt[3 * i + 1], tgt[3 * i + 2]);
      atomicAdd(&cell_count[cid], 1);
      atomicAdd(&th[cid / GS_GRID_TILE], 1);
    }
  }
  __syncthreads();
  for (int t = threadIdx.x; t < ntile; t += 256) {
    const int v = th[t];
    if (v) atomicAdd(&tile_sums[t], v);
  }
}
__global__ void __launch_bounds__(256) gs_grid_count_kernel(const float* __restrict__ tgt, GsCount n_tgt_c,
                                                            const GsTargetFilter flt,
                                                            const unsigned* __restrict__ bbox,
                                                            GsGrid* __restrict__ gp,
                                                            int* __restrict__ cell_count, int* __restrict__ tile_sums,
                                                            int cells_cap, const float4* __restrict__ tlist) {
  grid_count_body(tgt, gs_count(n_tgt_c), flt, bbox, gp, cell_count, tile_sums, cells_cap, tlist, blockIdx.x, gridDim.x);
}

GS_DEV void grid_scan_body(const int* __restrict__ cell_count, const GsGrid* __restrict__ gp,
                           const int* __restrict__ tile_sums, int* __restrict__ cell_start, const unsigned blk) {
  __shared__ int smem[256 / GS_WAVE + 1];
  const int n = gp->ncell + 1;
  if ((int)(blk * GS_GRID_TILE) >= n) return;
  int pre = 0;
  for (int t = threadIdx.x; t < (int)blk; t += 256) pre += tile_sums[t];
  int tile_prefix;
  (void)gs_block_excl_scan<256>(pre, smem, &tile_prefix);
  const int base = blk * GS_GRID_TILE + threadIdx.x * 4;
  int v[4], c = 0;
#pragma unroll
  for (int i = 0; i < 4; ++i) {
    v[i] = (base + i < n) ? cell_count[base + i] : 0;
    c += v[i];
  }
  int total;
  int run = tile_prefix + gs_block_excl_scan<256>(c, smem, &total);
#pragma unroll
  for (int i = 0; i < 4; ++i) {
    if (base + i < n) cell_start[base + i] = run;
    run += v[i];
  }
}
__global__ void __launch_bounds__(256) gs_grid_scan_kernel(const int* __restrict__ cell_count,
                                                           const GsGrid* __restrict__ gp,
                                                           const int* __restrict__ tile_sums,
                                                           int* __restrict__ cell_start) {
  grid_scan_body(cell_count, gp, tile_sums, cell_start, blockIdx.x);
}

GS_DEV void grid_scatter_body(const float* __restrict__ tgt, const int64_t n_tgt, const GsTargetFilter flt,
                              const GsGrid* __restrict__ gp, const int* __restrict__ cell_start,
                              int* __restrict__ cell_count, float4* __restrict__ sorted,
                              const float4* __restrict__ tlist, const unsigned* __restrict__ bbox,
                              const float* __restrict__ nrm, float4* __restrict__ sorted_n, const unsigned blk,
                              const unsigned nblk) {
  if (flt.pix) {
    const int64_t n_list = (int64_t)bbox[6];
    if ((int64_t)blk * 256 >= n_list) return;
    const GsGrid g = *gp;
    for (int64_t i = (int64_t)blk * 256 + threadIdx.x; i < n_list; i += (int64_t)nblk * 256) {
      const float4 t = tlist[i];
      const int cid = grid_cell(g, t.x, t.y, t.z);
      const int slot = cell_start[cid] + atomicSub(&cell_count[cid], 1) - 1;
      sorted[slot] = t;
      if (nrm) {
        const int64_t r = (int64_t)__float_as_int(t.w);
        sorted_n[slot] = make_float4(nrm[3 * r], nrm[3 * r + 1], nrm[3 * r + 2], 0.0f);
      }
    }
    return;
  }
  const int64_t i = (int64_t)blk * 256 + threadIdx.x;
  if (i >= n_tgt) return;
  const GsGrid g = *gp;
  const float x = tgt[3 * i], y = tgt[3 * i + 1], z = tgt[3 * i + 2];
  const int cid = grid_cell(g, x, y, z);
  const int slot = cell_start[cid] + atomicSub(&cell_count[cid], 1) - 1;
  sorted[slot] = make_float4(x, y, z, __int_as_float((int)i));
  if (nrm) sorted_n[slot] = make_float4(nrm[3 * i], nrm[3 * i + 1], nrm[3 * i + 2], 0.0f);
}
__global__ void __launch_bounds__(256) gs_grid_scatter_kernel(const float* __restrict__ tgt, GsCount n_tgt_c,
                                                              const GsTargetFilter flt,
                                                              const GsGrid* __restrict__ gp,
                                                              const int* __restrict__ cell_start,
                                                              int* __restrict__ cell_count,
                                                              float4* __restrict__ sorted,
                                                              const float4* __restrict__ tlist,
                                                              const unsigned* __restrict__ bbox,
                                                              const float* __restrict__ nrm,
                                                              float4* __restrict__ sorted_n) {
  grid_scatter_body(tgt, gs_count(n_tgt_c), flt, gp, cell_start, cell_count, sorted, tlist, bbox, nrm, sorted_n, blockIdx.x,
                    gridDim.x);
}

__global__ void __launch_bounds__(GB_BLOCK) gs_gridb_bbox_kernel(const GsGridBatch gb, float u_hi, float v_hi) {
  gridb_bbox_block(gb, blockIdx.x, u_hi, v_hi);
}
__global__ void __launch_bounds__(256) gs_gridb_count_kernel(const GsGridBatch gb) {
  const GsGridSeq& q = gb.s[blockIdx.x % gb.B];
  grid_count_body(q.tgt, gs_count(q.n_tgt), GsTargetFilter{q.pix, gb.W, gb.ds}, q.m.bbox, q.m.g, q.m.cell_count,
                  q.m.tile_sums, gb.cells_cap, q.m.tlist, blockIdx.x / gb.B, gridDim.x / gb.B);
}
__global__ void __launch_bounds__(256) gs_gridb_scan_kernel(const GsGridBatch gb) {
  const GsGridSeq& q = gb.s[blockIdx.x % gb.B];
  grid_scan_body(q.m.cell_count, q.m.g, q.m.tile_sums, q.m.cell_start, blockIdx.x / gb.B);
}
__global__ void __launch_bounds__(256) gs_gridb_scatter_kernel(const GsGridBatch gb) {
  const GsGridSeq& q = gb.s[blockIdx.x % gb.B];
  grid_scatter_body(q.tgt, gs_count(q.n_tgt), GsTargetFilter{q.pix, gb.W, gb.ds}, q.m.g, q.m.cell_start, q.m.cell_count,
                    q.m.sorted, q.m.tlist, q.m.bbox, q.nrm, q.m.sorted_n, blockIdx.x / gb.B, gridDim.x / gb.B);
}

static int grid_cells_cap(int64_t n_src, int64_t n_tgt_exact) {
  int64_t want = 48 * n_src;
  if (16 * n_tgt_exact > want) want = 16 * n_tgt_exact;
  int cells_cap = 1 << 20;
  while (cells_cap < GS_GRID_MAXCELL && cells_cap < want) cells_cap <<= 1;
  return cells_cap;
}
int gs_knn_grid_cells_cap(int64_t n_src) { return grid_cells_cap(n_src, 0); }
size_t gs_knn_grid_clear_bytes(const GridMem& m, int cells_cap) {
  return gs_align((size_t)(reinterpret_cast<char*>(m.cell_count) - reinterpret_cast<char*>(m.g)) +
                  4 * (size_t)(cells_cap + 1));
}

int gs_knn_grid_build_batch(const GsGridBatch& gb, hipStream_t st, bool bbox_done) {
  int64_t n_max = 1;
  for (int b = 0; b < gb.B; ++b) n_max = gb.s[b].n_tgt.host > n_max ? gb.s[b].n_tgt.host : n_max;
  const unsigned B = (unsigned)gb.B;
  const float u_hi = (float)((double)gb.W - 0.999), v_hi = (float)((double)gb.H - 0.999);
  if (!bbox_done)
    hipLaunchKernelGGL(gs_gridb_bbox_kernel, dim3(gs_knn_gridb_bbox_blocks(gb)), dim3(GB_BLOCK), 0, st, gb, u_hi, v_hi);
  bool listed = true;
  for (int b = 0; b < gb.B; ++b) listed = listed && gb.s[b].pix != nullptr;
  const int64_t slots = (int64_t)gs_ceil_div(gb.H, gb.ds) * gs_ceil_div(gb.W, gb.ds);
  unsigned nb_pts = (unsigned)gs_ceil_div(n_max, 256);
  if (listed && gb.H > 0 && (unsigned)gs_ceil_div(3 * slots, 256) < nb_pts) nb_pts = (unsigned)gs_ceil_div(3 * slots, 256);
  hipLaunchKernelGGL(gs_gridb_count_kernel, dim3(B * nb_pts), dim3(256), 0, st, gb);
  const unsigned ntile = (unsigned)gs_ceil_div(gb.cells_cap + 1, GS_GRID_TILE);
  hipLaunchKernelGGL(gs_gridb_scan_kernel, dim3(B * ntile), dim3(256), 0, st, gb);
  hipLaunchKernelGGL(gs_gridb_scatter_kernel, dim3(B * nb_pts), dim3(256), 0, st, gb);
  hipError_t e = hipGetLastError();
  if (e != hipSuccess) { gs_set_error("gs_knn_grid_build_batch: %s", hipGetErrorString(e)); return GS_ERR_HIP; }
  return GS_OK;
}

int gs_knn_grid_build(const float* tgt, GsCount n_tgt_c, int64_t n_src, void* grid_scratch, hipStream_t st,
                      GsTargetFilter flt, const float* nrm) {
  const int64_t n_tgt = n_tgt_c.host;
  GridMem m = grid_carve(grid_scratch, n_src, n_tgt);
  const int cells_cap = grid_cells_cap(n_src, n_tgt_c.dev ? 0 : n_tgt);
  GsProf prof(GS_PROF_COMPACT, 28.0 * (double)n_tgt + 8.0 * (double)cells_cap, st);
  const size_t clear = gs_knn_grid_clear_bytes(m, cells_cap);
  hipError_t e = hipMemsetAsync(m.g, 0, clear, st);
  if (e != hipSuccess) { gs_set_error("gs_knn_grid_build: %s", hipGetErrorString(e)); return GS_ERR_HIP; }
  hipLaunchKernelGGL(gs_grid_bbox_kernel, dim3((unsigned)gs_ceil_div(n_tgt > 0 ? n_tgt : 1, GB_BLOCK * GB_ITEMS)),
                     dim3(GB_BLOCK), 0, st, tgt, n_tgt_c, flt, m.bbox, m.unres_count, m.tlist);
  hipLaunchKernelGGL(gs_grid_count_kernel, dim3((unsigned)gs_ceil_div(n_tgt > 0 ? n_tgt : 1, 256)), dim3(256), 0, st,
                     tgt, n_tgt_c, flt, m.bbox, m.g, m.cell_count, m.tile_sums, cells_cap, m.tlist);
  const unsigned ntile = (unsigned)gs_ceil_div(cells_cap + 1, GS_GRID_TILE);
  hipLaunchKernelGGL(gs_grid_scan_kernel, dim3(ntile), dim3(256), 0, st, m.cell_count, m.g, m.tile_sums,
                     m.cell_start);
  hipLaunchKernelGGL(gs_grid_scatter_kernel, dim3((unsigned)gs_ceil_div(n_tgt, 256)), dim3(256), 0, st, tgt,
                     n_tgt_c, flt, m.g, m.cell_start, m.cell_count, m.sorted, m.tlist, m.bbox, nrm, m.sorted_n);
  return GS_OK;
}

constexpr int GQ_BLOCK = 256;

__global__ void __launch_bounds__(GQ_BLOCK) gs_grid_query_kernel(
    const float* __restrict__ src_in, const float* __restrict__ Tapply, float* __restrict__ src_out,
    int64_t n_src, const GsGrid* __restrict__ gp, const int* __restrict__ cell_start,
    const float4* __restrict__ sorted, unsigned long long* __restrict__ best, int* __restrict__ unres_count,
    int* __restrict__ unres_next, int* __restrict__ unres_list) {
  const int lane = threadIdx.x & (GQ_G - 1);
  const int64_t s = ((int64_t)blockIdx.x * GQ_BLOCK + threadIdx.x) / GQ_G;
  if (blockIdx.x == 0 && threadIdx.x == 0) *unres_next = 0;
  if (s >= n_src) return;
  const GsGrid g = *gp;
  float qx = src_in[3 * s], qy = src_in[3 * s + 1], qz = src_in[3 * s + 2];
  if (Tapply) {
    float T[12];
#pragma unroll
    for (int i = 0; i < 12; ++i) T[i] = Tapply[i];
    float t0, t1, t2;
    gs_rigid_fma(T, qx, qy, qz, t0, t1, t2);
    qx = t0; qy = t1; qz = t2;
  }
  if (src_out && lane == 0) {
    src_out[3 * s] = qx;
    src_out[3 * s + 1] = qy;
    src_out[3 * s + 2] = qz;
  }
  bool done;
  const unsigned long long key = grid_search_group(g, cell_start, sorted, qx, qy, qz, lane, &done);
  if (lane == 0) {
    if (done) {
      best[s] = key;
    } else {
      best[s] = ~0ull;
      unres_list[atomicAdd(unres_count, 1)] = (int)s;
    }
  }
}

int gs_knn_grid_query(const float* src_in, const float* Tapply, float* src_out, int64_t n_src,
                      const float* tgt, int64_t n_tgt, unsigned long long* best, void* grid_scratch,
                      hipStream_t st) {
  static unsigned seq = 0;
  GridMem m = grid_carve(grid_scratch, n_src, n_tgt);
  int* cnt = m.unres_count + (seq & 1);
  int* nxt = m.unres_count + ((seq + 1) & 1);
  ++seq;
  GsProf prof(GS_PROF_KNN, (double)n_src * (double)n_tgt, st);
  hipLaunchKernelGGL(gs_grid_query_kernel, dim3((unsigned)gs_ceil_div(n_src * GQ_G, GQ_BLOCK)), dim3(GQ_BLOCK), 0, st,
                     src_in, Tapply, src_out, n_src, m.g, m.cell_start, m.sorted, best, cnt, nxt, m.unres_list);
  unsigned gx = (unsigned)gs_ceil_div(n_src, KNN_BLOCK * 4);
  gx = gx > 4 ? 4 : gx;
  dim3 grid(gx, (unsigned)gs_ceil_div(n_tgt, KNN_TCHUNK));
  hipLaunchKernelGGL((gs_knn1_kernel<true, 4>), grid, dim3(KNN_BLOCK), 0, st, src_in, Tapply, nullptr, n_src, tgt,
                     n_tgt, best, m.unres_list, cnt);
  return GS_OK;
}

__global__ void __launch_bounds__(256) gs_knn_unpack_kernel(const unsigned long long* __restrict__ best,
                                                            int64_t n, int64_t n_tgt, int64_t* __restrict__ idx,
                                                            float* __restrict__ d2) {
  const int64_t i = (int64_t)blockIdx.x * 256 + threadIdx.x;
  if (i >= n) return;
  const unsigned long long b = best[i];
  int64_t j = (int64_t)(b & 0xffffffffull);
  if (j >= n_tgt) j = 0;
  idx[i] = j;
  if (d2) d2[i] = __uint_as_float((uint32_t)(b >> 32));
}

extern "C" int gs_knn1_f32(const float* src, int64_t n_src, const float* tgt, int64_t n_tgt,
                           int64_t* out_idx, float* out_d2, uint64_t* best_scratch, void* stream) {
  GS_REQUIRE(n_src > 0 && n_tgt > 0, "empty point set");
  GS_REQUIRE(n_tgt < 0x7fffffffll && n_src < 0x7fffffffll, "too many points");
  GS_REQUIRE(src && tgt && out_idx && best_scratch, "NULL pointer");
  hipStream_t st = gs_stream(stream);
  GS_HIP(hipMemsetAsync(best_scratch, 0xff, 8 * (size_t)n_src, st));
  gs_knn_brute_launch(src, nullptr, nullptr, n_src, tgt, n_tgt, reinterpret_cast<unsigned long long*>(best_scratch), st);
  hipLaunchKernelGGL(gs_knn_unpack_kernel, dim3((unsigned)gs_ceil_div(n_src, 256)), dim3(256), 0, st,
                     reinterpret_cast<const unsigned long long*>(best_scratch), n_src, n_tgt, out_idx, out_d2);
  GS_LAUNCH_CHECK();
  return GS_OK;
}

extern "C" int64_t gs_knn1_grid_scratch_bytes(int64_t n_src, int64_t n_tgt) {
  return (int64_t)(gs_align(8 * (size_t)(n_src > 0 ? n_src : 1)) + gs_knn_grid_scratch_bytes(n_src, n_tgt));
}

extern "C" int gs_knn1_grid_f32(const float* src, int64_t n_src, const float* tgt, int64_t n_tgt,
                                int64_t* out_idx, float* out_d2, void* scratch, int64_t* unresolved_out,
                                void* stream) {
  GS_REQUIRE(n_src > 0 && n_tgt > 0, "empty point set");
  GS_REQUIRE(n_tgt < 0x7fffffffll && n_src < 0x7fffffffll, "too many points");
  GS_REQUIRE(src && tgt && out_idx && scratch, "NULL pointer");
  hipStream_t st = gs_stream(stream);
  unsigned long long* best = reinterpret_cast<unsigned long long*>(scratch);
  void* gscratch = reinterpret_cast<char*>(scratch) + gs_align(8 * (size_t)n_src);
  GS_HIP(hipMemsetAsync(best, 0xff, 8 * (size_t)n_src, st));
  int rc = gs_knn_grid_build(tgt, GsCount{n_tgt, nullptr}, n_src, gscratch, st);
  if (rc != GS_OK) return rc;
  GridMem m = grid_carve(gscratch, n_src, n_tgt);
  rc = gs_knn_grid_query(src, nullptr, nullptr, n_src, tgt, n_tgt, best, gscratch, st);
  if (rc != GS_OK) return rc;
  hipLaunchKernelGGL(gs_knn_unpack_kernel, dim3((unsigned)gs_ceil_div(n_src, 256)), dim3(256), 0, st, best, n_src,
                     n_tgt, out_idx, out_d2);
  if (unresolved_out) {
    int h[2] = {0, 0};
    GS_HIP(hipMemcpyAsync(h, m.unres_count, 8, hipMemcpyDeviceToHost, st));
    GS_HIP(hipStreamSynchronize(st));
    *unresolved_out = (int64_t)h[0] + (int64_t)h[1];
  }
  GS_LAUNCH_CHECK();
  return GS_OK;
}
```

gradslam_amd/csrc/gs_knn_bbox.h:

```cpp
#pragma once
#include "gs_assoc_dev.h"
#include "gs_knn.h"

GS_DEV unsigned grid_code(float v) {
  const unsigned b = __float_as_uint(v);
  return (b & 0x80000000u) ? ~b : (b | 0x80000000u);
}
GS_DEV float grid_decode(unsigned c) {
  return __uint_as_float((c & 0x80000000u) ? (c & 0x7fffffffu) : ~c);
}
constexpr int GB_BLOCK = 256;
constexpr int GB_ITEMS = 8;
GS_DEV void grid_bbox_body(const float* __restrict__ tgt, const int64_t n_tgt, const GsTargetFilter flt,
                           const GsCamera* cam, int H, float u_hi, float v_hi, int32_t* __restrict__ pix_out,
                           unsigned* __restrict__ bbox, int* __restrict__ unres_count, float4* __restrict__ tlist,
                           const unsigned blk) {
  if (blk == 0 && threadIdx.x == 0) { unres_count[0] = 0; unres_count[1] = 0; }
  if ((int64_t)blk * GB_BLOCK * GB_ITEMS >= n_tgt) return;
  __shared__ float red[6][GB_BLOCK / GS_WAVE];
  __shared__ int scan_s[GB_BLOCK / GS_WAVE + 1];
  __shared__ unsigned base_s;
  int hits = 0;
  unsigned hitmask = 0;
  float lo[3] = {3.0e38f, 3.0e38f, 3.0e38f}, hi[3] = {-3.0e38f, -3.0e38f, -3.0e38f};
  const int64_t i0 = (int64_t)blk * GB_ITEMS * GB_BLOCK + threadIdx.x;
  if (cam) {
    float v[GB_ITEMS][3];
#pragma unroll
    for (int u = 0; u < GB_ITEMS; ++u) {
      const int64_t i = i0 + (int64_t)u * GB_BLOCK, ic = i < n_tgt ? i : n_tgt - 1;
      v[u][0] = tgt[3 * ic]; v[u][1] = tgt[3 * ic + 1]; v[u][2] = tgt[3 * ic + 2];
    }
#pragma unroll
    for (int u = 0; u < GB_ITEMS; ++u) {
      const int64_t i = i0 + (int64_t)u * GB_BLOCK;
      if (i < n_tgt) {
        int ph = 0, pw = 0;
        const bool in = gs_project_point_hw(*cam, v[u][0], v[u][1], v[u][2], H, flt.W, u_hi, v_hi, ph, pw);
        pix_out[i] = in ? (int32_t)(ph * flt.W + pw) : -1;
        if (in && gs_on_lattice(ph, pw, flt.ds)) {
          ++hits;
          hitmask |= 1u << u;
#pragma unroll
          for (int k = 0; k < 3; ++k) {
            const float w = v[u][k];
            if (w > -3.0e38f && w < 3.0e38f) {
              lo[k] = w < lo[k] ? w : lo[k];
              hi[k] = w > hi[k] ? w : hi[k];
            }
          }
        }
      }
    }
  } else {
    bool t[GB_ITEMS];
    if (flt.pix) {
      int32_t px[GB_ITEMS];
#pragma unroll
      for (int u = 0; u < GB_ITEMS; ++u) {
        const int64_t i = i0 + (int64_t)u * GB_BLOCK;
        px[u] = flt.pix[i < n_tgt ? i : n_tgt - 1];
      }
#pragma unroll
      for (int u = 0; u < GB_ITEMS; ++u) {
        const int32_t p = px[u];
        t[u] = (i0 + (int64_t)u * GB_BLOCK < n_tgt) && p >= 0 && ((p / flt.W) % flt.ds == 0) && ((p % flt.W) % flt.ds == 0);
      }
    } else {
#pragma unroll
      for (int u = 0; u < GB_ITEMS; ++u) t[u] = i0 + (int64_t)u * GB_BLOCK < n_tgt;
    }
#pragma unroll
    for (int u = 0; u < GB_ITEMS; ++u) {
      if (t[u]) {
        const int64_t i = i0 + (int64_t)u * GB_BLOCK;
        ++hits;
        hitmask |= 1u << u;
#pragma unroll
        for (int k = 0; k < 3; ++k) {
          const float w = tgt[3 * i + k];
          if (w > -3.0e38f && w < 3.0e38f) {
            lo[k] = w < lo[k] ? w : lo[k];
            hi[k] = w > hi[k] ? w : hi[k];
          }
        }
      }
    }
  }
  const int lane = threadIdx.x & 63, wave = threadIdx.x >> 6;
#pragma unroll
  for (int k = 0; k < 3; ++k) {
    float a = lo[k], b = hi[k];
#pragma unroll
    for (int d = 32; d > 0; d >>= 1) {
      const float a2 = __shfl_down(a, d, GS_WAVE), b2 = __shfl_down(b, d, GS_WAVE);
      a = a2 < a ? a2 : a;
      b = b2 > b ? b2 : b;
    }
    if (lane == 0) { red[k][wave] = a; red[3 + k][wave] = b; }
  }
  const bool filtered = flt.pix != nullptr || cam != nullptr;
  __syncthreads();
  if (filtered) {
    int total;
    int pos = gs_block_excl_scan<GB_BLOCK>(hits, scan_s, &total);
    if (threadIdx.x == 0 && total) base_s = atomicAdd(&bbox[6], (unsigned)total);
    __syncthreads();
    if (hitmask) {
      const unsigned base = base_s;
#pragma unroll
      for (int u = 0; u < GB_ITEMS; ++u) {
        if (hitmask & (1u << u)) {
          const int64_t i = ((int64_t)blk * GB_ITEMS + u) * GB_BLOCK + threadIdx.x;
          tlist[base + (unsigned)pos] = make_float4(tgt[3 * i], tgt[3 * i + 1], tgt[3 * i + 2], __int_as_float((int)i));
          ++pos;
        }
      }
    }
  }
  if (threadIdx.x < 3) {
    const int k = threadIdx.x;
    float a = red[k][0], b = red[3 + k][0];
    for (int w = 1; w < GB_BLOCK / GS_WAVE; ++w) {
      a = red[k][w] < a ? red[k][w] : a;
      b = red[3 + k][w] > b ? red[3 + k][w] : b;
    }
    if (a <= b) {
      atomicMax(&bbox[k], ~grid_code(a));
      atomicMax(&bbox[3 + k], grid_code(b));
    }
  }
}

GS_DEV void gridb_bbox_block(const GsGridBatch& gb, const unsigned bid, float u_hi, float v_hi) {
  const GsGridSeq& q = gb.s[bid % gb.B];
  const unsigned blk = bid / gb.B;
  const GsTargetFilter flt{q.pix, gb.W, gb.ds};
  if (q.pose16) {
    const GsCamera cam = gs_camera(q.pose16, q.K16);
    grid_bbox_body(q.tgt, gs_count(q.n_tgt), flt, &cam, gb.H, u_hi, v_hi, q.pix, q.m.bbox, q.m.unres_count, q.m.tlist,
                   blk);
  } else {
    grid_bbox_body(q.tgt, gs_count(q.n_tgt), flt, nullptr, 0, 0.0f, 0.0f, nullptr, q.m.bbox, q.m.unres_count, q.m.tlist,
                   blk);
  }
}
static inline unsigned gs_knn_gridb_bbox_blocks(const GsGridBatch& gb) {
  int64_t n_max = 1;
  for (int b = 0; b < gb.B; ++b) n_max = gb.s[b].n_tgt.host > n_max ? gb.s[b].n_tgt.host : n_max;
  return (unsigned)gb.B * (unsigned)gs_ceil_div(n_max, GB_BLOCK * GB_ITEMS);
}
```

gradslam_amd/slam/_fastpath.py:

```python
import os

import torch

from .. import _C, ops
from ..structures.pointclouds import _ATTRS
from .fusionutils import RENORMALIZE_UNMATCHED

__all__ = ["try_step"]

f32 = torch.float32
FASTPATH = os.environ.get("GRADSLAM_HIP_FASTPATH", "1") != "0"
STEP_GLOBAL_MAPS = os.environ.get("GRADSLAM_HIP_STEP_GLOBAL_MAPS", "0") == "1"


def _kwargs_key(kw):
    def norm(v):
        if torch.is_tensor(v):
            return ("tensor", id(v), int(v._version), tuple(v.shape), str(v.dtype), str(v.device))
        return v
    return tuple(sorted((k, norm(v)) for k, v in kw.items()))


def _dense_frames(t, inner):
    if t.dtype != f32 or t.stride()[2:] != inner:
        return None
    B = t.shape[0]
    sb = t.stride(0) if B > 1 else inner[0] * t.shape[2]
    if B > 1 and sb < inner[0] * t.shape[2]:
        return None
    return t.data_ptr(), sb


class StepPlan(object):
    def __init__(self, slam, B, H, W, device):
        self.B, self.H, self.W, self.P, self.device = B, H, W, H * W, device
        self.lib = _C.lib()
        self.seqs = (_C.StepSeq * B)()
        prov = slam.odomprov
        kw = prov._kwargs()
        self.kw_tensors = [v for v in kw.values() if torch.is_tensor(v)]
        self.prm = _C.IcpParams(int(prov._mode), int(kw.get("numiters", 20)), float(kw.get("damp", 1e-8)),
                                ops._thresh(kw.get("dist_thresh")), float(kw.get("lambda_max", 2.0)),
                                float(kw.get("B", 1.0)), float(kw.get("B2", 1.0)), float(kw.get("nu", 200.0)))
        self.key = (float(slam.sigma), float(slam.dist_th), float(slam.dot_th), int(slam.dsratio), _kwargs_key(kw),
                    int(prov._mode))
        self.sigma = float(slam.sigma)
        self.tss = ops.two_sigma_sq(slam.sigma)
        self.dist_th, self.dot_th, self.ds = float(slam.dist_th), float(slam.dot_th), int(slam.dsratio)
        self.caps = [-1] * B
        self.bufs = [None] * B
        self.scratch = [None] * B
        self.stream = _C.stream(device)
        self.stream_id = torch.cuda.current_stream(device).cuda_stream

    def _bind_map(self, pc, b):
        bufs = tuple(pc._buf[k][b] for k in _ATTRS)
        cap = int(bufs[0].shape[0])
        if any(t.shape[0] != cap for t in bufs):
            return False
        q = self.seqs[b]
        m = q.map
        m.points, m.normals, m.colors, m.ccounts = (t.data_ptr() for t in bufs)
        m.capacity = cap
        if cap != self.caps[b]:
            ws = _C.Workspace.get(self.device)
            loc = ws.bytes("localize%d" % b, self.lib.gs_localize_scratch_bytes(self.H, self.W, self.ds, cap))
            upd = ws.bytes("map_update%d" % b, self.lib.gs_update_map_scratch_bytes(cap, self.H, self.W))
            self.scratch[b] = (loc, upd)
            q.loc_scratch, q.upd_scratch = loc.data_ptr(), upd.data_ptr()
            self.caps[b] = cap
        self.bufs[b] = bufs
        return True

    def run(self, pc, live, prev):
        B, P, H, W = self.B, self.P, self.H, self.W
        dev = self.device
        d = _dense_frames(live._depth_image, (W, 1, 1))
        r = _dense_frames(live._rgb_image, (3 * W, 3, 1))
        K, pp = live._intrinsics, prev._poses
        if d is None or r is None or K.dtype != f32 or pp.dtype != f32 or not K.is_contiguous() or not pp.is_contiguous():
            return None
        grp = pc._dcount[0].group
        grp.poll()
        bounds = grp.bounds
        for b in range(B):
            bufs = self.bufs[b]
            if (bufs is None or any(bufs[i] is not pc._buf[k][b] for i, k in enumerate(_ATTRS)) or
                    bounds[b] + P > self.caps[b]):
                if bounds[b] + P > int(pc._buf["points"][b].shape[0]):
                    pc._reserve(b, P, pc.RESERVE_FRAMES)
                    bounds = grp.bounds
                if not self._bind_map(pc, b):
                    return None
        gm = STEP_GLOBAL_MAPS
        out = torch.empty(B * (13 if gm else 7) * P, dtype=f32, device=dev)
        poses_out = torch.empty(B * 16, dtype=f32, device=dev)
        best = torch.empty((B, P), dtype=torch.int32, device=dev)
        o = out.data_ptr()
        v0, n0, a0, po0 = o, o + 12 * P * B, o + 24 * P * B, poses_out.data_ptr()
        gv0, gn0 = o + 28 * P * B, o + 28 * P * B + 12 * P * B
        pair = getattr(grp, "_step_counts", None)
        if pair is None or pair[0].shape[0] != B or pair[0].device != dev:
            pair = grp._step_counts = [torch.zeros(B, dtype=torch.int64, device=dev) for _ in range(2)]
        cnt_new = pair[0] if pair[0].data_ptr() != grp.dev.data_ptr() else pair[1]
        d0, ds_ = d
        r0, rs_ = r
        k0, p0, c0, n_dev0, b0 = K.data_ptr(), pp.data_ptr(), cnt_new.data_ptr(), grp.dev.data_ptr(), best.data_ptr()
        seqs = self.seqs
        for b in range(B):
            q = seqs[b]
            q.depth, q.rgb = d0 + 4 * ds_ * b, r0 + 4 * rs_ * b
            q.K16, q.prev_pose16, q.out_pose16 = k0 + 64 * b, p0 + 64 * b, po0 + 64 * b
            q.vertex, q.normal, q.alpha = v0 + 12 * P * b, n0 + 12 * P * b, a0 + 4 * P * b
            q.gvertex, q.gnormal = (gv0 + 12 * P * b, gn0 + 12 * P * b) if gm else (None, None)
            q.best_pix = b0 + 4 * P * b
            q.new_count_out = c0 + 8 * b
            q.map.n_bound = bounds[b]
            q.map.n_dev = n_dev0 + 8 * b
        _C.check(self.lib.gs_pointfusion_step_batch_f32(seqs, B, H, W, self.ds, self.prm, self.tss, self.dist_th,
                                                        self.dot_th, 1 if RENORMALIZE_UNMATCHED else 0, self.stream), "gs_pointfusion_step_batch_f32")
        n3 = 3 * P * B
        live._vertex_map = out[:n3].view(B, 1, H, W, 3)
        live._normal_map = out[n3:2 * n3].view(B, 1, H, W, 3)
        live._alpha_cache = (self.sigma, out[2 * n3:2 * n3 + P * B].view(B, 1, H, W, 1))
        live._poses = poses_out.view(B, 1, 4, 4)
        if gm:
            g = 7 * P * B
            live._global_vertex_map = out[g:g + n3].view(B, 1, H, W, 3)
            live._global_normal_map = out[g + n3:g + 2 * n3].view(B, 1, H, W, 3)
        else:
            live._global_vertex_map = live._global_normal_map = None
        grp.advance(cnt_new, P)
        pc._generation += 1
        pc._padded_cache.clear()
        pc.equisized = True if B == 1 else None
        return pc, live._poses


def try_step(slam, pointclouds, live_frame, prev_frame):
    if not ops.DEVICE_COUNTS or not FASTPATH or prev_frame is None or slam.odom not in ("icp", "gradicp"):
        return None
    B = len(pointclouds._n_host)
    dc = pointclouds._dcount
    if B == 0 or len(dc) != B:
        return None
    g0 = dc[0].group
    if len(g0.bounds) != B or any(dc[b].group is not g0 or dc[b].index != b for b in range(B)) or min(g0.bounds) <= 0:
        return None
    if live_frame._channels_first or prev_frame._channels_first or live_frame._L != 1 or live_frame._B != B:
        return None
    if prev_frame._poses is None or live_frame._intrinsics.data_ptr() != prev_frame._intrinsics.data_ptr():
        return None
    if tuple(prev_frame._poses.shape) != (B, 1, 4, 4):
        return None
    dev = live_frame.device
    if dev.type != "cuda" or pointclouds.device != dev or prev_frame.device != dev:
        return None
    bufs = pointclouds._buf
    if any(bufs[k] is None for k in _ATTRS) or bufs["points"][0].dtype != f32 or bufs["features"][0].shape[-1] != 1:
        return None
    if torch.is_grad_enabled() and (live_frame._depth_image.requires_grad or live_frame._rgb_image.requires_grad or
                                    prev_frame._poses.requires_grad or
                                    any(t.requires_grad for k in _ATTRS for t in bufs[k])):
        return None
    from ..odometry.gradicp import GradICPOdometryProvider
    from ..odometry.icp import ICPOdometryProvider
    if type(slam.odomprov) not in (ICPOdometryProvider, GradICPOdometryProvider):
        return None
    H, W = live_frame.h, live_frame.w
    plan = getattr(slam, "_step_plan", None)
    key = (float(slam.sigma), float(slam.dist_th), float(slam.dot_th), int(slam.dsratio),
           _kwargs_key(slam.odomprov._kwargs()), int(slam.odomprov._mode))
    if (plan is None or (plan.B, plan.H, plan.W, plan.device) != (B, H, W, dev) or plan.key != key or
            plan.stream_id != torch.cuda.current_stream(dev).cuda_stream):
        plan = slam._step_plan = StepPlan(slam, B, H, W, dev)
    return plan.run(pointclouds, live_frame, prev_frame)
```

include/gradslam_hip.h:

```cpp
#ifndef GRADSLAM_HIP_H
#define GRADSLAM_HIP_H

#include <stdint.h>

#ifdef __cplusplus
extern "C" {
#endif

#define GS_API __attribute__((visibility("default")))

#define GS_OK 0
#define GS_ERR_INVALID 1
#define GS_ERR_HIP 2
#define GS_ERR_CAPACITY 3

GS_API int gs_abi_version(void);
GS_API const char* gs_last_error(void);
GS_API int64_t gs_scratch_bytes(int64_t n_map, int64_t n_pix);

GS_API int gs_profile_begin(int max_records);
GS_API int gs_profile_end(void);
GS_API int gs_profile_read(int kind, double* ms_total, int64_t* launches, double* work_total);

GS_API int gs_frame_maps_f32(const float* depth, const float* K16, int H, int W, float two_sigma_sq,
                      float* vertex, float* normal, float* alpha, uint8_t* valid, void* stream);

GS_API int gs_global_maps_f32(const float* vertex, const float* normal, const float* depth,
                       const float* pose16, int H, int W, float* gvertex, float* gnormal,
                       void* stream);

GS_API int gs_alpha_f32(const float* points, int64_t n, float two_sigma_sq, float eps, float* alpha,
                 void* stream);

GS_API int gs_alpha_backward_f32(const float* points, int64_t n, float two_sigma_sq, float eps,
                          const float* alpha_bar, float* points_bar, float* sigma_terms, void* stream);

GS_API int gs_downsample_frame_f32(const float* gvertex, const float* gnormal, const float* rgb,
                            const float* depth, int H, int W, int ds, float* out_pts,
                            float* out_nrm, float* out_rgb, int64_t* count_out, void* scratch,
                            void* stream);

GS_API int gs_project_map_f32(const float* points, int64_t n_map, const float* pose16,
                       const float* K16, int H, int W, int32_t* pix, void* stream);

GS_API int gs_active_table_i64(const int32_t* pix, int64_t n_map, int W, int64_t b, int64_t* rows_out,
                        int64_t* count_out, void* scratch, void* stream);

GS_API int gs_select_targets_f32(const int32_t* pix, int64_t n_map, int W, int ds, const float* points,
                          const float* normals, const float* colors, float* out_pts,
                          float* out_nrm, float* out_rgb, int64_t cap, int64_t* count_out,
                          void* scratch, void* stream);

GS_API int gs_downsample_table_f32(const int64_t* rows, int64_t n_rows, int ds, const float* points,
                            const float* normals, const float* colors, float* out_pts,
                            float* out_nrm, float* out_rgb, int64_t* count_out, void* scratch,
                            void* stream);

GS_API int gs_knn1_f32(const float* src, int64_t n_src, const float* tgt, int64_t n_tgt,
                int64_t* out_idx, float* out_d2, uint64_t* best_scratch, void* stream);

GS_API int64_t gs_knn1_grid_scratch_bytes(int64_t n_src, int64_t n_tgt);
GS_API int gs_knn1_grid_f32(const float* src, int64_t n_src, const float* tgt, int64_t n_tgt,
                            int64_t* out_idx, float* out_d2, void* scratch, int64_t* unresolved_out_host,
                            void* stream);

GS_API int gs_gauss_newton_rows_f32(const float* src, int64_t n_src, const float* tgt,
                             const float* tgt_normals, int64_t n_tgt, float dist_thresh,
                             float* A, float* b, int64_t* idx, uint8_t* keep,
                             uint64_t* best_scratch, void* stream);

GS_API int gs_solve_normal_eq_f32(const float* A, const float* b, const uint8_t* keep, int64_t n_rows,
                           int ncols, float damp, float* x, void* stream);

GS_API int gs_se3_exp_f32(const float* xi6, float* T16, void* stream);

GS_API int gs_se3_exp_backward_f32(const float* xi6, const float* Tbar16, float* xi_bar6, void* stream);

GS_API int gs_relative_pose_f32(const float* T01, const float* T02, int64_t n, float* out, void* stream);

GS_API int gs_transform_points_f32(const float* pts, int64_t n, const float* T16, float* out,
                            void* stream);

typedef struct gs_icp_params {
  int mode;
  int numiters;
  float damp;
  float dist_thresh;
  float lambda_max;
  float B;
  float B2;
  float nu;
} gs_icp_params;

GS_API int64_t gs_icp_scratch_bytes(int64_t n_src, int64_t n_tgt);
GS_API int gs_icp_f32(const float* src, int64_t n_src, const float* tgt, const float* tgt_normals,
               int64_t n_tgt, const float* init16, const float* compose16,
               const gs_icp_params* params_host, float* out_T16, int64_t* out_idx,
               void* icp_scratch, void* stream);

GS_API int64_t gs_frame_maps_backward_kbar_scratch_bytes(int H, int W);
GS_API int gs_frame_maps_backward_f32(const float* depth, const float* K16, int H, int W, float two_sigma_sq,
                                      const float* vertex_bar, const float* normal_bar, const float* alpha_bar,
                                      float* depth_bar, float* scratch_6hw, float* K_bar16, void* kbar_scratch,
                                      void* stream);
GS_API int gs_global_maps_backward_f32(const float* gvertex_bar, const float* gnormal_bar, const float* depth,
                                       const float* pose16, int H, int W, float* vertex_bar, float* normal_bar,
                                       void* stream);
GS_API int64_t gs_global_maps_pose_backward_scratch_bytes(int H, int W);
GS_API int gs_global_maps_pose_backward_f32(const float* vertex, const float* normal, const float* depth,
                                            const float* gvertex_bar, const float* gnormal_bar, int H, int W,
                                            float* pose_bar16, void* scratch, void* stream);
GS_API int gs_downsample_frame_backward_f32(const float* pts_bar, const float* depth, int H, int W, int ds,
                                            float* gvertex_bar, void* scratch, void* stream);

GS_API int64_t gs_icp_tape_bytes(int64_t n_src, int numiters);
GS_API int gs_icp_tape_f32(const float* src, int64_t n_src, const float* tgt, const float* tgt_normals,
                           int64_t n_tgt, const float* init16, const float* compose16,
                           const gs_icp_params* params_host, float* out_T16, int64_t* out_idx,
                           void* icp_scratch, void* tape, void* stream);
GS_API int64_t gs_icp_backward_scratch_bytes(int64_t n_src, int64_t n_tgt);
GS_API int gs_icp_backward_f32(const void* tape, const float* src, int64_t n_src, const float* tgt,
                               const float* tgt_normals, int64_t n_tgt, const float* init16,
                               const gs_icp_params* params_host, const float* T_bar16, float* src_bar,
                               float* tgt_bar, float* normals_bar, float* init_bar16, void* scratch,
                               void* stream);

GS_API int gs_icp_dc_f32(const float* src, int64_t n_src_bound, const int64_t* n_src_dev, const float* tgt,
                         const float* tgt_normals, int64_t n_tgt_bound, const int64_t* n_tgt_dev,
                         const float* init16, const float* compose16, const gs_icp_params* params_host,
                         float* out_T16, int64_t* out_idx, void* icp_scratch, void* stream);

GS_API int gs_icp_map_dc_f32(const float* src, int64_t n_src_bound, const int64_t* n_src_dev,
                             const float* map_points, const float* map_normals, const int32_t* pix,
                             int64_t n_map_bound, const int64_t* n_map_dev, int W, int ds, const float* init16,
                             const float* compose16, const gs_icp_params* params_host, float* out_T16,
                             void* icp_scratch, void* stream);

GS_API int gs_icp_trace_f32(const void* icp_scratch, int numiters, float* trace_out, void* stream);

GS_API int gs_similar_rows_f32(const int64_t* rows, int64_t n_rows, const float* points,
                        const float* normals, const float* gvertex, const float* gnormal, int W,
                        float dist_th, float dot_th, uint8_t* mask, void* stream);

GS_API int gs_best_unique_rows_f32(const int64_t* rows, int64_t n_rows, const float* points,
                            const float* ccounts, const float* gvertex, int H, int W, int64_t b,
                            int32_t* best_pix, int64_t* rows_out, int64_t* count_out,
                            void* scratch, void* stream);

GS_API int gs_associate_f32(const int32_t* pix, int64_t n_map, const float* points,
                     const float* normals, const float* ccounts, const float* gvertex,
                     const float* gnormal, int H, int W, float dist_th, float dot_th,
                     int32_t* best_pix, uint8_t* similar, void* scratch, void* stream);

GS_API int gs_best_table_i64(const int32_t* best_pix, int H, int W, int64_t b, int64_t* rows_out,
                      int64_t* count_out, void* scratch, void* stream);
GS_API int gs_rows_to_best_pix(const int64_t* rows, int64_t n_rows, int H, int W, int32_t* best_pix,
                        void* stream);

GS_API int gs_fuse_append_f32(float* points, float* normals, float* colors, float* ccounts,
                       int64_t n_map_host, int64_t capacity, const int32_t* best_pix,
                       const float* gvertex, const float* gnormal, const float* rgb,
                       const float* alpha, const float* depth, int H, int W, int renorm_all,
                       int64_t* new_count_out, void* scratch, void* stream);

GS_API int gs_append_valid_f32(float* points, float* normals, float* colors, float* ccounts,
                        int64_t n_map_host, int64_t capacity, const float* gvertex,
                        const float* gnormal, const float* rgb, const float* alpha,
                        const float* depth, int H, int W, int64_t* new_count_out, void* scratch,
                        void* stream);

GS_API int gs_lattice_source_f32(const float* vertex, const float* depth, const float* pose16, int H, int W, int ds,
                                 float* out_pts, void* stream);

GS_API int gs_ingest_depth_u16_f32(const uint16_t* raw, int H0, int W0, float* out, int H, int W,
                                   double scale_div, void* stream);
GS_API int gs_ingest_color_u8_f32(const uint8_t* raw, int H0, int W0, float* out, int H, int W, int normalize,
                                  void* stream);
GS_API int gs_ingest_frames_native_f32(const uint16_t* depth_raw, const uint8_t* color_raw, int64_t n_frames, int H, int W,
                                       double scale_div, int normalize, float* depth_out, float* color_out, void* stream);
GS_API int gs_host_device_pointer(const void* host_ptr, void** dev_ptr_out);

GS_API int gs_project_map_dc_f32(const float* points, int64_t n_map_bound, const int64_t* n_map_dev,
                                 const float* pose16, const float* K16, int H, int W, int32_t* pix,
                                 void* stream);
GS_API int gs_select_targets_dc_f32(const int32_t* pix, int64_t n_map_bound, const int64_t* n_map_dev, int W,
                                    int ds, const float* points, const float* normals, const float* colors,
                                    float* out_pts, float* out_nrm, float* out_rgb, int64_t cap,
                                    int64_t* count_out, void* scratch, void* stream);
GS_API int gs_associate_dc_f32(const int32_t* pix, int64_t n_map_bound, const int64_t* n_map_dev,
                               const float* points, const float* normals, const float* ccounts,
                               const float* gvertex, const float* gnormal, int H, int W, float dist_th,
                               float dot_th, int32_t* best_pix, uint8_t* similar, void* scratch, void* stream);
GS_API int gs_fuse_append_dc_f32(float* points, float* normals, float* colors, float* ccounts,
                                 int64_t n_map_bound, const int64_t* n_map_dev, int64_t capacity,
                                 const int32_t* best_pix, const float* gvertex, const float* gnormal,
                                 const float* rgb, const float* alpha, const float* depth, int H, int W,
                                 int renorm_all, int64_t* new_count_out, void* scratch, void* stream);
GS_API int gs_append_valid_dc_f32(float* points, float* normals, float* colors, float* ccounts,
                                  int64_t n_map_bound, const int64_t* n_map_dev, int64_t capacity,
                                  const float* gvertex, const float* gnormal, const float* rgb,
                                  const float* alpha, const float* depth, int H, int W,
                                  int64_t* new_count_out, void* scratch, void* stream);

GS_API int gs_fuse_append_backward_f32(const float* points, const float* normals, const float* colors,
                                       const float* ccounts, int64_t n_old, const int32_t* best_pix,
                                       const float* gvertex, const float* gnormal, const float* rgb,
                                       const float* alpha, const float* depth, int H, int W, int renorm_all,
                                       const float* P_bar, const float* N_bar, const float* C_bar,
                                       const float* F_bar, int64_t n_new, float* old_points_bar,
                                       float* old_normals_bar, float* old_colors_bar, float* old_ccounts_bar,
                                       float* gvertex_bar, float* gnormal_bar, float* rgb_bar, float* alpha_bar,
                                       void* scratch, void* stream);

GS_API int64_t gs_update_map_scratch_bytes(int64_t n_map_bound, int H, int W);
GS_API int gs_update_map_fusion_dc_f32(float* points, float* normals, float* colors, float* ccounts,
                                       int64_t n_map_bound, const int64_t* n_map_dev, int64_t capacity,
                                       const float* vertex, const float* normal, const float* depth,
                                       const float* rgb, const float* alpha, const float* pose16, const float* K16,
                                       int H, int W, float dist_th, float dot_th, int renorm_all, float* gvertex,
                                       float* gnormal, int32_t* best_pix, int64_t* new_count_out, void* scratch,
                                       void* stream);

typedef struct gs_map_view {
  float* points;
  float* normals;
  float* colors;
  float* ccounts;
  int64_t capacity;
  int64_t n_bound;
  const int64_t* n_dev;
} gs_map_view;

GS_API int gs_frame_maps_batch_f32(const float* depth, int64_t depth_stride_seq, int64_t depth_stride_frame,
                                   const float* K16, int n_frames, int frames_per_K, int H, int W, float two_sigma_sq,
                                   float* vertex, float* normal, float* alpha, void* stream);

typedef struct gs_localize_seq {
  const float* vertex;
  const float* depth;
  const float* K16;
  const float* prev_pose16;
  gs_map_view map;
  float* out_pose16;
  void* scratch;
} gs_localize_seq;
GS_API int64_t gs_localize_scratch_bytes(int H, int W, int ds, int64_t n_map_bound);
GS_API int gs_localize_batch_f32(const gs_localize_seq* seqs_host, int B, int H, int W, int ds,
                                 const gs_icp_params* params_host, void* stream);
GS_API int gs_localize_far_stats_i64(const void* scratch, int H, int W, int ds, int64_t map_rows, int64_t* out4_host,
                                     void* stream);
GS_API int gs_localize_list_stats_i64(const void* scratch, int H, int W, int ds, int64_t map_rows, int64_t* out192_host,
                                      void* stream);
GS_API int gs_localize_solve_stats_i64(const void* scratch, int H, int W, int ds, int64_t map_rows, int64_t* out8_host,
                                       void* stream);

typedef struct gs_update_seq {
  gs_map_view map;
  const float* vertex;
  const float* normal;
  const float* depth;
  const float* rgb;
  const float* alpha;
  const float* pose16;
  const float* K16;
  float* gvertex;
  float* gnormal;
  int32_t* best_pix;
  int64_t* new_count_out;
  void* scratch;
} gs_update_seq;
GS_API int gs_update_map_fusion_batch_f32(const gs_update_seq* seqs_host, int B, int H, int W, float dist_th,
                                          float dot_th, int renorm_all, void* stream);

typedef struct gs_step_seq {
  const float* depth;
  const float* rgb;
  const float* K16;
  const float* prev_pose16;
  float* out_pose16;
  float* vertex;
  float* normal;
  float* alpha;
  float* gvertex;
  float* gnormal;
  int32_t* best_pix;
  int64_t* new_count_out;
  gs_map_view map;
  void* loc_scratch;
  void* upd_scratch;
} gs_step_seq;
GS_API int gs_pointfusion_step_batch_f32(const gs_step_seq* seqs_host, int B, int H, int W, int ds,
                                         const gs_icp_params* params_host, float two_sigma_sq, float dist_th,
                                         float dot_th, int renorm_all, void* stream);

GS_API int gs_project_points_f32(const float* cam_coords, int cdim, int64_t n, const float* proj16, int64_t pts_per_mat,
                                 float* out_uv, void* stream);
GS_API int gs_unproject_points_f32(const float* pixel_coords, int pdim, int64_t n, const float* kinv9,
                                   int64_t pts_per_mat, const float* depths, float* out_xyz, void* stream);
GS_API int gs_lie_small_f32(int op, const float* in, float* out, void* stream);

typedef struct gs_render_seq {
  gs_map_view map;
  const float* poses16;
  const float* K16;
  float* depth;
  float* color;
  float* normal;
  float* confidence;
  int64_t* index;
  void* scratch;
} gs_render_seq;
GS_API int64_t gs_render_scratch_bytes(int views, int H, int W);
GS_API int gs_render_map_dc_f32(const gs_render_seq* seqs_host, int B, int L, int H, int W, int radius,
                                float min_confidence, int cull_backfaces, void* stream);

typedef struct gs_render_backward_seq {
  gs_map_view map;
  const float* poses16;
  const float* K16;
  const int64_t* index;
  const float* depth_bar;
  const float* color_bar;
  const float* normal_bar;
  const float* confidence_bar;
  float* points_bar;
  float* normals_bar;
  float* colors_bar;
  float* ccounts_bar;
  float* poses_bar;
  void* scratch;
} gs_render_backward_seq;
GS_API int64_t gs_render_backward_scratch_bytes(int views, int H, int W, int64_t n_bound);
GS_API int gs_render_map_backward_dc_f32(const gs_render_backward_seq* seqs_host, int B, int L, int H, int W,
                                         int radius, void* stream);

#ifdef __cplusplus
}
#endif
#endif
```

Before: 3880.

## Skip KNN grid count clearing when scratch is retained clean across frames

```diff
diff --git a/gradslam_amd/_C.py b/gradslam_amd/_C.py
--- a/gradslam_amd/_C.py
+++ b/gradslam_amd/_C.py
@@ -79,6 +79,8 @@
     "gs_knn1_f32": [_vp, _i64, _vp, _i64, _vp, _vp, _vp, _vp],
     "gs_knn1_grid_scratch_bytes": [_i64, _i64],
     "gs_knn1_grid_f32": [_vp, _i64, _vp, _i64, _vp, _vp, _vp, C.POINTER(C.c_int64), _vp],
+    "gs_knn1_grid_retained_f32": [_vp, _i64, _vp, _i64, _vp, _vp, _vp, _i32, C.POINTER(C.c_int64), _vp],
+    "gs_knn1_grid_counts_range": [_i64, _i64, C.POINTER(C.c_int64), C.POINTER(C.c_int64)],
     "gs_gauss_newton_rows_f32": [_vp, _i64, _vp, _vp, _i64, _f, _vp, _vp, _vp, _vp, _vp, _vp],
     "gs_solve_normal_eq_f32": [_vp, _vp, _vp, _i64, _i32, _f, _vp, _vp],
     "gs_se3_exp_f32": [_vp, _vp, _vp],
@@ -138,6 +140,8 @@
     "gs_localize_list_stats_i64": [_vp, _i32, _i32, _i32, _i64, C.POINTER(C.c_int64), _vp],
     "gs_localize_solve_stats_i64": [_vp, _i32, _i32, _i32, _i64, C.POINTER(C.c_int64), _vp],
     "gs_pointfusion_step_batch_f32": [C.POINTER(StepSeq), _i32, _i32, _i32, _i32, C.POINTER(IcpParams), _f, _f, _f, _i32, _vp],
+    "gs_pointfusion_step_batch_retained_f32": [C.POINTER(StepSeq), _i32, _i32, _i32, _i32, C.POINTER(IcpParams), _f, _f, _f, _i32,
+                                               _i32, _vp],
     "gs_render_scratch_bytes": [_i32, _i32, _i32],
     "gs_render_map_dc_f32": [C.POINTER(RenderSeq), _i32, _i32, _i32, _i32, _i32, _f, _i32, _vp],
     "gs_render_backward_scratch_bytes": [_i32, _i32, _i32, _i64],
diff --git a/gradslam_amd/csrc/gs_icp_loop.hip b/gradslam_amd/csrc/gs_icp_loop.hip
--- a/gradslam_amd/csrc/gs_icp_loop.hip
+++ b/gradslam_amd/csrc/gs_icp_loop.hip
@@ -1453,7 +1453,7 @@
 }
 
 static void loc_bind(const gs_localize_seq* seqs, int B, int H, int W, int ds, const gs_icp_params* prm,
-                     const IcpEnginePlan& plan, LocCarve* c, LocBatch& lb, GsGridBatch& gb) {
+                     const IcpEnginePlan& plan, LocCarve* c, LocBatch& lb, GsGridBatch& gb, bool counts_clean) {
   lb.B = gb.B = B; lb.W = gb.W = W; gb.H = H; lb.ds = gb.ds = ds;
   lb.Wl = (W + ds - 1) / ds; lb.n_lat = loc_lattice(H, W, ds); lb.damp = prm->damp; lb.numiters = prm->numiters;
   gb.cells_cap = gs_knn_grid_cells_cap(lb.n_lat);
@@ -1467,7 +1467,7 @@
                         plan.binned_normals ? q.map.normals : nullptr, c[b].gm};
   }
   lb.count_valid = g_gs_prof_on ? 1 : 0;
-  lb.clear_bytes = gs_knn_grid_clear_bytes(c[0].gm, gb.cells_cap);
+  lb.clear_bytes = gs_knn_grid_clear_bytes(c[0].gm, gb.cells_cap, counts_clean);
 }
 
 static int loc_prep(const gs_localize_seq* seqs, const LocBatch& lb, const GsGridBatch& gb, hipStream_t st, bool grid_cleared) {
@@ -1583,8 +1583,18 @@
   hipLaunchKernelGGL(gs_icp_finish_batch_kernel, dim3((unsigned)B), dim3(FS_BLOCK), 0, st, fb, GsCount{n_lat, nullptr}, h & 1, *prm);
 }
 
+static GsScratchSig loc_sig(int H, int W, int ds, const gs_map_view& map) {
+  const int64_t n_lat = loc_lattice(H, W, ds);
+  return GsScratchSig{1, gs_knn_grid_cells_cap(n_lat), n_lat, loc_rows(map)};
+}
+static bool loc_counts_clean(const gs_localize_seq* seqs, int B, int H, int W, int ds) {
+  for (int b = 0; b < B; ++b)
+    if (!gs_scratch_counts_clean(seqs[b].scratch, loc_sig(H, W, ds, seqs[b].map))) return false;
+  return true;
+}
+
 static int localize_chunk(const gs_localize_seq* seqs, int B, int H, int W, int ds, const gs_icp_params* prm,
-                          hipStream_t st, bool grid_cleared) {
+                          hipStream_t st, bool grid_cleared, bool counts_clean) {
   const int64_t n_lat = loc_lattice(H, W, ds);
   LocLayout layouts[GS_MAX_BATCH]; LocCarve c[GS_MAX_BATCH];
   for (int b = 0; b < B; ++b) {
@@ -1593,10 +1603,15 @@
   }
   const IcpEnginePlan plan = icp_engine_plan(gs_env(), icp_device(), B, n_lat, prm->numiters, layouts);
   LocBatch lb; GsGridBatch gb;
-  loc_bind(seqs, B, H, W, ds, prm, plan, c, lb, gb);
+  loc_bind(seqs, B, H, W, ds, prm, plan, c, lb, gb, counts_clean);
+  for (int b = 0; b < B; ++b) gs_scratch_mark(seqs[b].scratch, loc_sig(H, W, ds, seqs[b].map), false);
   int rc = loc_prep(seqs, lb, gb, st, grid_cleared);
   if (rc != GS_OK) return rc;
-  if (prm->numiters == 0) { GS_LAUNCH_CHECK(); return GS_OK; }
+  if (prm->numiters == 0) {
+    GS_LAUNCH_CHECK();
+    for (int b = 0; b < B; ++b) gs_scratch_mark(seqs[b].scratch, loc_sig(H, W, ds, seqs[b].map), true);
+    return GS_OK;
+  }
   double prof_bytes = 0.0;
   if (g_gs_prof_on && (rc = loc_prof_bytes(B, c, n_lat, prm->numiters, st, &prof_bytes)) != GS_OK) return rc;
   {
@@ -1606,11 +1621,12 @@
   }
   loc_finish(seqs, B, plan, c, n_lat, prm, st);
   GS_LAUNCH_CHECK();
+  for (int b = 0; b < B; ++b) gs_scratch_mark(seqs[b].scratch, loc_sig(H, W, ds, seqs[b].map), true);
   return GS_OK;
 }
 
 static int localize_batch(const gs_localize_seq* seqs_host, int B, int H, int W, int ds, const gs_icp_params* prm,
-                          void* stream, bool grid_cleared) {
+                          void* stream, bool grid_cleared, bool counts_clean) {
   GS_REQUIRE(seqs_host && prm && B > 0 && H > 0 && W > 0 && ds > 0, "bad arguments");
   GS_REQUIRE(prm->numiters >= 0 && prm->numiters <= GS_ICP_MAX_ITERS, "numiters must be in [0, 1024]");
   GS_REQUIRE(prm->mode == 0 || prm->mode == 1, "mode must be 0 (ICP) or 1 (gradICP)");
@@ -1625,14 +1641,14 @@
   hipStream_t st = gs_stream(stream);
   for (int c0 = 0; c0 < B; c0 += GS_MAX_BATCH) {
     const int nb = B - c0 < GS_MAX_BATCH ? B - c0 : GS_MAX_BATCH;
-    const int rc = localize_chunk(seqs_host + c0, nb, H, W, ds, prm, st, grid_cleared);
+    const int rc = localize_chunk(seqs_host + c0, nb, H, W, ds, prm, st, grid_cleared, counts_clean);
     if (rc != GS_OK) return rc;
   }
   return GS_OK;
 }
 extern "C" int gs_localize_batch_f32(const gs_localize_seq* seqs_host, int B, int H, int W, int ds,
                                      const gs_icp_params* prm, void* stream) {
-  return localize_batch(seqs_host, B, H, W, ds, prm, stream, false);
+  return localize_batch(seqs_host, B, H, W, ds, prm, stream, false, false);
 }
 
 __global__ void __launch_bounds__(256) gs_far_stats_kernel(const int* __restrict__ far_idx, const int* __restrict__ far_n,
@@ -1697,9 +1713,9 @@
   return GS_OK;
 }
 
-extern "C" int gs_pointfusion_step_batch_f32(const gs_step_seq* seqs_host, int B, int H, int W, int ds,
-                                             const gs_icp_params* prm, float two_sigma_sq, float dist_th, float dot_th,
-                                             int renorm_all, void* stream) {
+extern "C" int gs_pointfusion_step_batch_retained_f32(const gs_step_seq* seqs_host, int B, int H, int W, int ds,
+                                                      const gs_icp_params* prm, float two_sigma_sq, float dist_th,
+                                                      float dot_th, int renorm_all, int scratch_retained, void* stream) {
   GS_REQUIRE(seqs_host && prm && B > 0 && H > 0 && W > 0 && ds > 0, "bad arguments");
   const int64_t P = (int64_t)H * W;
   const gs_step_seq& s0 = seqs_host[0];
@@ -1734,11 +1750,12 @@
     }
     GsClearJob job;
     job.n = nb;
+    const bool counts_clean = scratch_retained != 0 && loc_counts_clean(ls, nb, H, W, ds);
     for (int b = 0; b < nb; ++b) {
       GS_REQUIRE(ls[b].map.points && ls[b].map.n_bound > 0, "every sequence needs a non-empty map");
       const LocCarve cv = loc_carve_of(ls[b].scratch, H, W, ds, loc_rows(ls[b].map));
       job.ptr[b] = reinterpret_cast<char*>(cv.gm.g);
-      if (b == 0) job.bytes = gs_knn_grid_clear_bytes(cv.gm, gs_knn_grid_cells_cap(loc_lattice(H, W, ds)));
+      if (b == 0) job.bytes = gs_knn_grid_clear_bytes(cv.gm, gs_knn_grid_cells_cap(loc_lattice(H, W, ds)), counts_clean);
     }
     GsPixelTables tabs{};
     tabs.n = implicit_global ? nb : 0;
@@ -1750,10 +1767,16 @@
     int rc = gs_frame_maps_batch_clear(sq[0].depth, dstride, P, sq[0].K16, nb, 1, H, W, two_sigma_sq, sq[0].vertex,
                                        sq[0].normal, sq[0].alpha, &job, stream, &tabs);
     if (rc != GS_OK) return rc;
-    rc = localize_batch(ls, nb, H, W, ds, prm, stream, true);
+    rc = localize_batch(ls, nb, H, W, ds, prm, stream, true, counts_clean);
     if (rc != GS_OK) return rc;
   }
   return gs_update_map_fusion_batch_impl(us.get(), B, H, W, dist_th, dot_th, renorm_all, stream, implicit_global);
+}
+extern "C" int gs_pointfusion_step_batch_f32(const gs_step_seq* seqs_host, int B, int H, int W, int ds,
+                                             const gs_icp_params* prm, float two_sigma_sq, float dist_th, float dot_th,
+                                             int renorm_all, void* stream) {
+  return gs_pointfusion_step_batch_retained_f32(seqs_host, B, H, W, ds, prm, two_sigma_sq, dist_th, dot_th, renorm_all, 0,
+                                                stream);
 }
 
 extern "C" int64_t gs_icp_tape_bytes(int64_t n_src, int numiters) { return (int64_t)gs_icp_tape_size(n_src, numiters); }
diff --git a/gradslam_amd/csrc/gs_knn.h b/gradslam_amd/csrc/gs_knn.h
--- a/gradslam_amd/csrc/gs_knn.h
+++ b/gradslam_amd/csrc/gs_knn.h
@@ -29,6 +29,7 @@
   return p >= 0 && ((p / f.W) % f.ds == 0) && ((p % f.W) % f.ds == 0);
 }
 
+constexpr int GS_BBOX_TICKET = 8, GS_COUNT_TICKET = 9;
 struct GridMem {
   GsGrid* g;
   unsigned* bbox;
@@ -76,11 +77,19 @@
   GsGridSeq s[GS_MAX_BATCH];
 };
 int gs_knn_grid_cells_cap(int64_t n_src);
-size_t gs_knn_grid_clear_bytes(const GridMem& m, int cells_cap);
+size_t gs_knn_grid_clear_bytes(const GridMem& m, int cells_cap, bool counts_clean = false);
+struct GsScratchSig {
+  int kind;
+  int cells_cap;
+  int64_t a, b;
+};
+bool gs_scratch_counts_clean(const void* base, const GsScratchSig& sig);
+void gs_scratch_mark(const void* base, const GsScratchSig& sig, bool clean);
 int gs_knn_grid_build_batch(const GsGridBatch& gb, hipStream_t st, bool bbox_done = false);
 
 int gs_knn_grid_build(const float* tgt, GsCount n_tgt, int64_t n_src, void* grid_scratch, hipStream_t st,
-                      GsTargetFilter filter = GsTargetFilter{nullptr, 1, 1}, const float* nrm = nullptr);
+                      GsTargetFilter filter = GsTargetFilter{nullptr, 1, 1}, const float* nrm = nullptr,
+                      bool counts_clean = false);
 int gs_knn_grid_query(const float* src_in, const float* Tapply, float* src_out, int64_t n_src,
                       const float* tgt, int64_t n_tgt, unsigned long long* best, void* grid_scratch,
                       hipStream_t st);
diff --git a/gradslam_amd/csrc/gs_knn.hip b/gradslam_amd/csrc/gs_knn.hip
--- a/gradslam_amd/csrc/gs_knn.hip
+++ b/gradslam_amd/csrc/gs_knn.hip
@@ -1,6 +1,9 @@
 #include "gs_knn.h"
 
 #include <stdlib.h>
+
+#include <mutex>
+#include <unordered_map>
 
 #include "gs_assoc_dev.h"
 #include "gs_env.h"
@@ -108,100 +111,95 @@
                                                                  const GsTargetFilter flt,
                                                                  unsigned* __restrict__ bbox,
                                                                  int* __restrict__ unres_count,
-                                                                 float4* __restrict__ tlist) {
-  grid_bbox_body(tgt, gs_count(n_tgt_c), flt, nullptr, 0, 0.0f, 0.0f, nullptr, bbox, unres_count, tlist, blockIdx.x);
-}
-
-GS_DEV GsGrid grid_from_bbox(const unsigned* __restrict__ bbox, int64_t n_tgt, int cells_cap) {
-  float o[3], m[3];
-#pragma unroll
-  for (int k = 0; k < 3; ++k) {
-    const unsigned cl = bbox[k], ch = bbox[3 + k];
-    float a = 0.0f, b = 0.0f;
-    if (cl != 0u && ch != 0u) { a = grid_decode(~cl); b = grid_decode(ch); }
-    o[k] = a; m[k] = b;
-  }
-  const float tiny = 1e-6f;
-  const float ex = (m[0] - o[0]) + tiny, ey = (m[1] - o[1]) + tiny, ez = (m[2] - o[2]) + tiny;
-  const float n = (float)(n_tgt > 0 ? n_tgt : 1);
-  const float area = ex * ey + ey * ez + ex * ez;
-  float c = 1.5f * sqrtf(area / n);
-  const float cv = 0.5f * cbrtf((ex * ey * ez) / n);
-  c = cv > c ? cv : c;
-  const float emax = ex > ey ? (ex > ez ? ex : ez) : (ey > ez ? ey : ez);
-  c = c > emax * (1.0f / 1024.0f) ? c : emax * (1.0f / 1024.0f);
-  c = c > 1e-6f ? c : 1e-6f;
-  int nx, ny, nz;
-  for (;;) {
-    nx = (int)(ex / c) + 1; ny = (int)(ey / c) + 1; nz = (int)(ez / c) + 1;
-    if ((double)nx * (double)ny * (double)nz <= (double)cells_cap) break;
-    c *= 1.26f;
-  }
-  GsGrid g;
-  g.ox = o[0]; g.oy = o[1]; g.oz = o[2];
-  g.mx = m[0]; g.my = m[1]; g.mz = m[2];
-  g.c = c; g.inv_c = 1.0f / c;
-  g.nx = nx; g.ny = ny; g.nz = nz; g.ncell = nx * ny * nz;
-  return g;
-}
-
+                                                                 float4* __restrict__ tlist, GsGrid* __restrict__ gp,
+                                                                 int cells_cap) {
+  grid_bbox_body(tgt, gs_count(n_tgt_c), flt, nullptr, 0, 0.0f, 0.0f, nullptr, bbox, unres_count, tlist, gp, cells_cap,
+                 blockIdx.x);
+}
+
+constexpr int GC_HASH = 512;
+static_assert(GC_HASH >= 2 * 256 && (GC_HASH & (GC_HASH - 1)) == 0, "a pass of 256 targets must fit the hash half empty");
 GS_DEV void grid_count_body(const float* __restrict__ tgt, const int64_t n_tgt, const GsTargetFilter flt,
-                            const unsigned* __restrict__ bbox, GsGrid* __restrict__ gp, int* __restrict__ cell_count,
-                            int* __restrict__ tile_sums, int cells_cap, const float4* __restrict__ tlist,
-                            const unsigned blk, const unsigned nblk) {
-  __shared__ GsGrid gsh;
-  __shared__ int th[GS_GRID_MAXCELL / GS_GRID_TILE + 1];
+                            unsigned* __restrict__ bbox, const GsGrid* __restrict__ gp, int* __restrict__ cell_count,
+                            int* __restrict__ tile_sums, const float4* __restrict__ tlist, const unsigned blk,
+                            const unsigned nblk) {
+  __shared__ int hk[GC_HASH], hv[GC_HASH];
+  __shared__ int smem[256 / GS_WAVE + 1];
+  __shared__ bool last_s;
   const int64_t n_items = flt.pix ? (int64_t)bbox[6] : n_tgt;
   if ((int64_t)blk * 256 >= n_items && blk != 0) return;
+  const GsGrid g = *gp;
+  for (int t = threadIdx.x; t < GC_HASH; t += 256) { hk[t] = -1; hv[t] = 0; }
+  __syncthreads();
+  for (int64_t base = (int64_t)blk * 256; base < n_items; base += (int64_t)nblk * 256) {
+    const int64_t i = base + threadIdx.x;
+    if (i < n_items) {
+      float x, y, z;
+      if (flt.pix) { const float4 t = tlist[i]; x = t.x; y = t.y; z = t.z; }
+      else { x = tgt[3 * i]; y = tgt[3 * i + 1]; z = tgt[3 * i + 2]; }
+      const int cid = grid_cell(g, x, y, z);
+      atomicAdd(&cell_count[cid], 1);
+      const int tile = cid / GS_GRID_TILE;
+      for (int h = tile & (GC_HASH - 1);; h = (h + 1) & (GC_HASH - 1)) {
+        const int was = atomicCAS(&hk[h], -1, tile);
+        if (was == -1 || was == tile) { atomicAdd(&hv[h], 1); break; }
+      }
+    }
+    __syncthreads();
+    for (int t = threadIdx.x; t < GC_HASH; t += 256) {
+      const int v = hv[t];
+      if (v) { atomicAdd(&tile_sums[hk[t]], v); hk[t] = -1; hv[t] = 0; }
+    }
+    __syncthreads();
+  }
+  __threadfence();
+  __syncthreads();
   if (threadIdx.x == 0) {
-    gsh = grid_from_bbox(bbox, n_items, cells_cap);
-    if (blk == 0) *gp = gsh;
+    const int64_t want = (n_items + 255) / 256;
+    const unsigned nact = want < 1 ? 1u : (want < (int64_t)nblk ? (unsigned)want : nblk);
+    last_s = atomicAdd(&bbox[GS_COUNT_TICKET], 1u) == nact - 1;
   }
   __syncthreads();
-  const GsGrid g = gsh;
-  const int ntile = g.ncell / GS_GRID_TILE + 1;
-  for (int t = threadIdx.x; t < ntile; t += 256) th[t] = 0;
-  __syncthreads();
-  if (flt.pix) {
-    for (int64_t i = (int64_t)blk * 256 + threadIdx.x; i < n_items; i += (int64_t)nblk * 256) {
-      const float4 t = tlist[i];
-      const int cid = grid_cell(g, t.x, t.y, t.z);
-      atomicAdd(&cell_count[cid], 1);
-      atomicAdd(&th[cid / GS_GRID_TILE], 1);
-    }
-  } else {
-    const int64_t i = (int64_t)blk * 256 + threadIdx.x;
-    if (i < n_tgt) {
-      const int cid = grid_cell(g, tgt[3 * i], tgt[3 * i + 1], tgt[3 * i + 2]);
-      atomicAdd(&cell_count[cid], 1);
-      atomicAdd(&th[cid / GS_GRID_TILE], 1);
-    }
-  }
-  __syncthreads();
-  for (int t = threadIdx.x; t < ntile; t += 256) {
-    const int v = th[t];
-    if (v) atomicAdd(&tile_sums[t], v);
+  if (!last_s) return;
+  __threadfence();
+  const int n_ent = g.ncell / GS_GRID_TILE + 2;
+  const int per = (n_ent + 255) / 256, e0 = threadIdx.x * per;
+  int c = 0;
+  for (int e = e0; e < e0 + per && e < n_ent - 1; ++e)
+    c += __hip_atomic_load(&tile_sums[e], __ATOMIC_RELAXED, __HIP_MEMORY_SCOPE_AGENT);
+  int total;
+  int run = gs_block_excl_scan<256>(c, smem, &total);
+  for (int e = e0; e < e0 + per && e < n_ent; ++e) {
+    const int v = e < n_ent - 1 ? __hip_atomic_load(&tile_sums[e], __ATOMIC_RELAXED, __HIP_MEMORY_SCOPE_AGENT) : 0;
+    tile_sums[e] = run;
+    run += v;
   }
 }
 __global__ void __launch_bounds__(256) gs_grid_count_kernel(const float* __restrict__ tgt, GsCount n_tgt_c,
-                                                            const GsTargetFilter flt,
-                                                            const unsigned* __restrict__ bbox,
-                                                            GsGrid* __restrict__ gp,
+                                                            const GsTargetFilter flt, unsigned* __restrict__ bbox,
+                                                            const GsGrid* __restrict__ gp,
                                                             int* __restrict__ cell_count, int* __restrict__ tile_sums,
-                                                            int cells_cap, const float4* __restrict__ tlist) {
-  grid_count_body(tgt, gs_count(n_tgt_c), flt, bbox, gp, cell_count, tile_sums, cells_cap, tlist, blockIdx.x, gridDim.x);
+                                                            const float4* __restrict__ tlist) {
+  grid_count_body(tgt, gs_count(n_tgt_c), flt, bbox, gp, cell_count, tile_sums, tlist, blockIdx.x, gridDim.x);
 }
 
 GS_DEV void grid_scan_body(const int* __restrict__ cell_count, const GsGrid* __restrict__ gp,
-                           const int* __restrict__ tile_sums, int* __restrict__ cell_start, const unsigned blk) {
+                           const int* __restrict__ tile_pre, int* __restrict__ cell_start, const unsigned blk) {
   __shared__ int smem[256 / GS_WAVE + 1];
   const int n = gp->ncell + 1;
   if ((int)(blk * GS_GRID_TILE) >= n) return;
-  int pre = 0;
-  for (int t = threadIdx.x; t < (int)blk; t += 256) pre += tile_sums[t];
-  int tile_prefix;
-  (void)gs_block_excl_scan<256>(pre, smem, &tile_prefix);
+  const int tile_prefix = tile_pre[blk];
+  const bool empty = tile_pre[blk + 1] == tile_prefix;
   const int base = blk * GS_GRID_TILE + threadIdx.x * 4;
+  if (empty) {
+    if (base + 3 < n) {
+      *reinterpret_cast<int4*>(cell_start + base) = make_int4(tile_prefix, tile_prefix, tile_prefix, tile_prefix);
+    } else {
+      for (int i = 0; i < 4; ++i)
+        if (base + i < n) cell_start[base + i] = tile_prefix;
+    }
+    return;
+  }
   int v[4], c = 0;
 #pragma unroll
   for (int i = 0; i < 4; ++i) {
@@ -216,6 +214,7 @@
     run += v[i];
   }
 }
+static_assert(GS_GRID_TILE == 4 * 256, "a scan block of 256 threads takes four cells per thread");
 __global__ void __launch_bounds__(256) gs_grid_scan_kernel(const int* __restrict__ cell_count,
                                                            const GsGrid* __restrict__ gp,
                                                            const int* __restrict__ tile_sums,
@@ -274,7 +273,7 @@
 __global__ void __launch_bounds__(256) gs_gridb_count_kernel(const GsGridBatch gb) {
   const GsGridSeq& q = gb.s[blockIdx.x % gb.B];
   grid_count_body(q.tgt, gs_count(q.n_tgt), GsTargetFilter{q.pix, gb.W, gb.ds}, q.m.bbox, q.m.g, q.m.cell_count,
-                  q.m.tile_sums, gb.cells_cap, q.m.tlist, blockIdx.x / gb.B, gridDim.x / gb.B);
+                  q.m.tile_sums, q.m.tlist, blockIdx.x / gb.B, gridDim.x / gb.B);
 }
 __global__ void __launch_bounds__(256) gs_gridb_scan_kernel(const GsGridBatch gb) {
   const GsGridSeq& q = gb.s[blockIdx.x % gb.B];
@@ -294,9 +293,23 @@
   return cells_cap;
 }
 int gs_knn_grid_cells_cap(int64_t n_src) { return grid_cells_cap(n_src, 0); }
-size_t gs_knn_grid_clear_bytes(const GridMem& m, int cells_cap) {
-  return gs_align((size_t)(reinterpret_cast<char*>(m.cell_count) - reinterpret_cast<char*>(m.g)) +
-                  4 * (size_t)(cells_cap + 1));
+size_t gs_knn_grid_clear_bytes(const GridMem& m, int cells_cap, bool counts_clean) {
+  const size_t front = (size_t)(reinterpret_cast<char*>(m.cell_count) - reinterpret_cast<char*>(m.g));
+  return gs_align(front + (counts_clean ? 0 : 4 * (size_t)(cells_cap + 1)));
+}
+
+static std::mutex g_scratch_mu;
+static std::unordered_map<const void*, GsScratchSig> g_scratch_clean;
+bool gs_scratch_counts_clean(const void* base, const GsScratchSig& sig) {
+  std::lock_guard<std::mutex> lk(g_scratch_mu);
+  const auto it = g_scratch_clean.find(base);
+  return it != g_scratch_clean.end() && it->second.kind == sig.kind && it->second.cells_cap == sig.cells_cap &&
+         it->second.a == sig.a && it->second.b == sig.b;
+}
+void gs_scratch_mark(const void* base, const GsScratchSig& sig, bool clean) {
+  std::lock_guard<std::mutex> lk(g_scratch_mu);
+  if (clean) g_scratch_clean[base] = sig;
+  else g_scratch_clean.erase(base);
 }
 
 int gs_knn_grid_build_batch(const GsGridBatch& gb, hipStream_t st, bool bbox_done) {
@@ -321,23 +334,26 @@
 }
 
 int gs_knn_grid_build(const float* tgt, GsCount n_tgt_c, int64_t n_src, void* grid_scratch, hipStream_t st,
-                      GsTargetFilter flt, const float* nrm) {
+                      GsTargetFilter flt, const float* nrm, bool counts_clean) {
   const int64_t n_tgt = n_tgt_c.host;
   GridMem m = grid_carve(grid_scratch, n_src, n_tgt);
   const int cells_cap = grid_cells_cap(n_src, n_tgt_c.dev ? 0 : n_tgt);
   GsProf prof(GS_PROF_COMPACT, 28.0 * (double)n_tgt + 8.0 * (double)cells_cap, st);
-  const size_t clear = gs_knn_grid_clear_bytes(m, cells_cap);
+  const size_t clear = gs_knn_grid_clear_bytes(m, cells_cap, counts_clean);
   hipError_t e = hipMemsetAsync(m.g, 0, clear, st);
   if (e != hipSuccess) { gs_set_error("gs_knn_grid_build: %s", hipGetErrorString(e)); return GS_ERR_HIP; }
+  const unsigned nb_pts = (unsigned)gs_ceil_div(n_tgt > 0 ? n_tgt : 1, 256);
   hipLaunchKernelGGL(gs_grid_bbox_kernel, dim3((unsigned)gs_ceil_div(n_tgt > 0 ? n_tgt : 1, GB_BLOCK * GB_ITEMS)),
-                     dim3(GB_BLOCK), 0, st, tgt, n_tgt_c, flt, m.bbox, m.unres_count, m.tlist);
-  hipLaunchKernelGGL(gs_grid_count_kernel, dim3((unsigned)gs_ceil_div(n_tgt > 0 ? n_tgt : 1, 256)), dim3(256), 0, st,
-                     tgt, n_tgt_c, flt, m.bbox, m.g, m.cell_count, m.tile_sums, cells_cap, m.tlist);
+                     dim3(GB_BLOCK), 0, st, tgt, n_tgt_c, flt, m.bbox, m.unres_count, m.tlist, m.g, cells_cap);
+  hipLaunchKernelGGL(gs_grid_count_kernel, dim3(nb_pts), dim3(256), 0, st, tgt, n_tgt_c, flt, m.bbox, m.g, m.cell_count,
+                     m.tile_sums, m.tlist);
   const unsigned ntile = (unsigned)gs_ceil_div(cells_cap + 1, GS_GRID_TILE);
   hipLaunchKernelGGL(gs_grid_scan_kernel, dim3(ntile), dim3(256), 0, st, m.cell_count, m.g, m.tile_sums,
                      m.cell_start);
-  hipLaunchKernelGGL(gs_grid_scatter_kernel, dim3((unsigned)gs_ceil_div(n_tgt, 256)), dim3(256), 0, st, tgt,
-                     n_tgt_c, flt, m.g, m.cell_start, m.cell_count, m.sorted, m.tlist, m.bbox, nrm, m.sorted_n);
+  hipLaunchKernelGGL(gs_grid_scatter_kernel, dim3(nb_pts), dim3(256), 0, st, tgt, n_tgt_c, flt, m.g, m.cell_start,
+                     m.cell_count, m.sorted, m.tlist, m.bbox, nrm, m.sorted_n);
+  e = hipGetLastError();
+  if (e != hipSuccess) { gs_set_error("gs_knn_grid_build: %s", hipGetErrorString(e)); return GS_ERR_HIP; }
   return GS_OK;
 }
 
@@ -393,7 +409,8 @@
   unsigned gx = (unsigned)gs_ceil_div(n_src, KNN_BLOCK * 4);
   gx = gx > 4 ? 4 : gx;
   dim3 grid(gx, (unsigned)gs_ceil_div(n_tgt, KNN_TCHUNK));
-  hipLaunchKernelGGL((gs_knn1_kernel<true, 4>), grid, dim3(KNN_BLOCK), 0, st, src_in, Tapply, nullptr, n_src, tgt,
+  if (n_tgt > 0)
+    hipLaunchKernelGGL((gs_knn1_kernel<true, 4>), grid, dim3(KNN_BLOCK), 0, st, src_in, Tapply, nullptr, n_src, tgt,
                      n_tgt, best, m.unres_list, cnt);
   return GS_OK;
 }
@@ -428,18 +445,22 @@
   return (int64_t)(gs_align(8 * (size_t)(n_src > 0 ? n_src : 1)) + gs_knn_grid_scratch_bytes(n_src, n_tgt));
 }
 
-extern "C" int gs_knn1_grid_f32(const float* src, int64_t n_src, const float* tgt, int64_t n_tgt,
-                                int64_t* out_idx, float* out_d2, void* scratch, int64_t* unresolved_out,
-                                void* stream) {
-  GS_REQUIRE(n_src > 0 && n_tgt > 0, "empty point set");
+extern "C" int gs_knn1_grid_retained_f32(const float* src, int64_t n_src, const float* tgt, int64_t n_tgt,
+                                         int64_t* out_idx, float* out_d2, void* scratch, int scratch_retained,
+                                         int64_t* unresolved_out, void* stream) {
+  GS_REQUIRE(n_src > 0 && n_tgt >= 0, "empty query set");
   GS_REQUIRE(n_tgt < 0x7fffffffll && n_src < 0x7fffffffll, "too many points");
-  GS_REQUIRE(src && tgt && out_idx && scratch, "NULL pointer");
+  GS_REQUIRE(src && (tgt || n_tgt == 0) && out_idx && scratch, "NULL pointer");
   hipStream_t st = gs_stream(stream);
   unsigned long long* best = reinterpret_cast<unsigned long long*>(scratch);
   void* gscratch = reinterpret_cast<char*>(scratch) + gs_align(8 * (size_t)n_src);
+  const GsScratchSig sig{0, grid_cells_cap(n_src, n_tgt), n_src, n_tgt};
+  const bool clean = scratch_retained != 0 && gs_scratch_counts_clean(scratch, sig);
+  gs_scratch_mark(scratch, sig, false);
   GS_HIP(hipMemsetAsync(best, 0xff, 8 * (size_t)n_src, st));
-  int rc = gs_knn_grid_build(tgt, GsCount{n_tgt, nullptr}, n_src, gscratch, st);
+  int rc = gs_knn_grid_build(tgt, GsCount{n_tgt, nullptr}, n_src, gscratch, st, GsTargetFilter{nullptr, 1, 1}, nullptr, clean);
   if (rc != GS_OK) return rc;
+  gs_scratch_mark(scratch, sig, true);
   GridMem m = grid_carve(gscratch, n_src, n_tgt);
   rc = gs_knn_grid_query(src, nullptr, nullptr, n_src, tgt, n_tgt, best, gscratch, st);
   if (rc != GS_OK) return rc;
@@ -454,3 +475,18 @@
   GS_LAUNCH_CHECK();
   return GS_OK;
 }
+
+extern "C" int gs_knn1_grid_f32(const float* src, int64_t n_src, const float* tgt, int64_t n_tgt,
+                                int64_t* out_idx, float* out_d2, void* scratch, int64_t* unresolved_out,
+                                void* stream) {
+  GS_REQUIRE(n_src > 0 && n_tgt > 0, "empty point set");
+  return gs_knn1_grid_retained_f32(src, n_src, tgt, n_tgt, out_idx, out_d2, scratch, 0, unresolved_out, stream);
+}
+
+extern "C" int gs_knn1_grid_counts_range(int64_t n_src, int64_t n_tgt, int64_t* offset_bytes, int64_t* n_words) {
+  GS_REQUIRE(n_src > 0 && n_tgt >= 0 && offset_bytes && n_words, "bad arguments");
+  const GridMem m = grid_carve(reinterpret_cast<void*>((uintptr_t)4096), n_src, n_tgt);
+  *offset_bytes = (int64_t)gs_align(8 * (size_t)n_src) + (reinterpret_cast<char*>(m.cell_count) - reinterpret_cast<char*>(m.g));
+  *n_words = (int64_t)grid_cells_cap(n_src, n_tgt) + 1;
+  return GS_OK;
+}
diff --git a/gradslam_amd/csrc/gs_knn_bbox.h b/gradslam_amd/csrc/gs_knn_bbox.h
--- a/gradslam_amd/csrc/gs_knn_bbox.h
+++ b/gradslam_amd/csrc/gs_knn_bbox.h
@@ -9,13 +9,49 @@
 GS_DEV float grid_decode(unsigned c) {
   return __uint_as_float((c & 0x80000000u) ? (c & 0x7fffffffu) : ~c);
 }
+GS_DEV GsGrid grid_from_bbox(const unsigned* __restrict__ bbox, int64_t n_tgt, int cells_cap) {
+  float o[3], m[3];
+#pragma unroll
+  for (int k = 0; k < 3; ++k) {
+    const unsigned cl = bbox[k], ch = bbox[3 + k];
+    float a = 0.0f, b = 0.0f;
+    if (cl != 0u && ch != 0u) { a = grid_decode(~cl); b = grid_decode(ch); }
+    o[k] = a; m[k] = b;
+  }
+  const float tiny = 1e-6f;
+  const float ex = (m[0] - o[0]) + tiny, ey = (m[1] - o[1]) + tiny, ez = (m[2] - o[2]) + tiny;
+  const float n = (float)(n_tgt > 0 ? n_tgt : 1);
+  const float area = ex * ey + ey * ez + ex * ez;
+  float c = 1.5f * sqrtf(area / n);
+  const float cv = 0.5f * cbrtf((ex * ey * ez) / n);
+  c = cv > c ? cv : c;
+  const float emax = ex > ey ? (ex > ez ? ex : ez) : (ey > ez ? ey : ez);
+  c = c > emax * (1.0f / 1024.0f) ? c : emax * (1.0f / 1024.0f);
+  c = c > 1e-6f ? c : 1e-6f;
+  int nx, ny, nz;
+  for (;;) {
+    nx = (int)(ex / c) + 1; ny = (int)(ey / c) + 1; nz = (int)(ez / c) + 1;
+    if ((double)nx * (double)ny * (double)nz <= (double)cells_cap) break;
+    c *= 1.26f;
+  }
+  GsGrid g;
+  g.ox = o[0]; g.oy = o[1]; g.oz = o[2];
+  g.mx = m[0]; g.my = m[1]; g.mz = m[2];
+  g.c = c; g.inv_c = 1.0f / c;
+  g.nx = nx; g.ny = ny; g.nz = nz; g.ncell = nx * ny * nz;
+  return g;
+}
+
 constexpr int GB_BLOCK = 256;
 constexpr int GB_ITEMS = 8;
 GS_DEV void grid_bbox_body(const float* __restrict__ tgt, const int64_t n_tgt, const GsTargetFilter flt,
                            const GsCamera* cam, int H, float u_hi, float v_hi, int32_t* __restrict__ pix_out,
                            unsigned* __restrict__ bbox, int* __restrict__ unres_count, float4* __restrict__ tlist,
-                           const unsigned blk) {
-  if (blk == 0 && threadIdx.x == 0) { unres_count[0] = 0; unres_count[1] = 0; }
+                           GsGrid* __restrict__ gp, const int cells_cap, const unsigned blk) {
+  if (blk == 0 && threadIdx.x == 0) {
+    unres_count[0] = 0; unres_count[1] = 0;
+    if (n_tgt <= 0) *gp = grid_from_bbox(bbox, 0, cells_cap);
+  }
   if ((int64_t)blk * GB_BLOCK * GB_ITEMS >= n_tgt) return;
   __shared__ float red[6][GB_BLOCK / GS_WAVE];
   __shared__ int scan_s[GB_BLOCK / GS_WAVE + 1];
@@ -130,6 +166,18 @@
       atomicMax(&bbox[3 + k], grid_code(b));
     }
   }
+  __threadfence();
+  __syncthreads();
+  if (threadIdx.x == 0) {
+    const unsigned nblk = (unsigned)((n_tgt + GB_BLOCK * GB_ITEMS - 1) / (GB_BLOCK * GB_ITEMS));
+    if (atomicAdd(&bbox[GS_BBOX_TICKET], 1u) == nblk - 1) {
+      __threadfence();
+      unsigned fin[7];
+#pragma unroll
+      for (int k = 0; k < 7; ++k) fin[k] = __hip_atomic_load(&bbox[k], __ATOMIC_RELAXED, __HIP_MEMORY_SCOPE_AGENT);
+      *gp = grid_from_bbox(fin, filtered ? (int64_t)fin[6] : n_tgt, cells_cap);
+    }
+  }
 }
 
 GS_DEV void gridb_bbox_block(const GsGridBatch& gb, const unsigned bid, float u_hi, float v_hi) {
@@ -139,10 +187,10 @@
   if (q.pose16) {
     const GsCamera cam = gs_camera(q.pose16, q.K16);
     grid_bbox_body(q.tgt, gs_count(q.n_tgt), flt, &cam, gb.H, u_hi, v_hi, q.pix, q.m.bbox, q.m.unres_count, q.m.tlist,
-                   blk);
+                   q.m.g, gb.cells_cap, blk);
   } else {
     grid_bbox_body(q.tgt, gs_count(q.n_tgt), flt, nullptr, 0, 0.0f, 0.0f, nullptr, q.m.bbox, q.m.unres_count, q.m.tlist,
-                   blk);
+                   q.m.g, gb.cells_cap, blk);
   }
 }
 static inline unsigned gs_knn_gridb_bbox_blocks(const GsGridBatch& gb) {
diff --git a/gradslam_amd/slam/_fastpath.py b/gradslam_amd/slam/_fastpath.py
--- a/gradslam_amd/slam/_fastpath.py
+++ b/gradslam_amd/slam/_fastpath.py
@@ -50,6 +50,9 @@
         self.caps = [-1] * B
         self.bufs = [None] * B
         self.scratch = [None] * B
+        self.ws_bufs = _C.Workspace.get(device)._bufs
+        self.loc_names = ["localize%d" % b for b in range(B)]
+        self.vouched = False
         self.stream = _C.stream(device)
         self.stream_id = torch.cuda.current_stream(device).cuda_stream
 
@@ -67,6 +70,7 @@
             loc = ws.bytes("localize%d" % b, self.lib.gs_localize_scratch_bytes(self.H, self.W, self.ds, cap))
             upd = ws.bytes("map_update%d" % b, self.lib.gs_update_map_scratch_bytes(cap, self.H, self.W))
             self.scratch[b] = (loc, upd)
+            self.vouched = False
             q.loc_scratch, q.upd_scratch = loc.data_ptr(), upd.data_ptr()
             self.caps[b] = cap
         self.bufs[b] = bufs
@@ -85,6 +89,8 @@
         bounds = grp.bounds
         for b in range(B):
             bufs = self.bufs[b]
+            if self.scratch[b] is not None and self.ws_bufs.get(self.loc_names[b]) is not self.scratch[b][0]:
+                self.caps[b], bufs = -1, None
             if (bufs is None or any(bufs[i] is not pc._buf[k][b] for i, k in enumerate(_ATTRS)) or
                     bounds[b] + P > self.caps[b]):
                 if bounds[b] + P > int(pc._buf["points"][b].shape[0]):
@@ -117,8 +123,12 @@
             q.new_count_out = c0 + 8 * b
             q.map.n_bound = bounds[b]
             q.map.n_dev = n_dev0 + 8 * b
-        _C.check(self.lib.gs_pointfusion_step_batch_f32(seqs, B, H, W, self.ds, self.prm, self.tss, self.dist_th,
-                                                        self.dot_th, 1 if RENORMALIZE_UNMATCHED else 0, self.stream), "gs_pointfusion_step_batch_f32")
+        retained, self.vouched = self.vouched, False
+        _C.check(self.lib.gs_pointfusion_step_batch_retained_f32(seqs, B, H, W, self.ds, self.prm, self.tss, self.dist_th,
+                                                                 self.dot_th, 1 if RENORMALIZE_UNMATCHED else 0,
+                                                                 1 if retained else 0, self.stream),
+                 "gs_pointfusion_step_batch_retained_f32")
+        self.vouched = True
         n3 = 3 * P * B
         live._vertex_map = out[:n3].view(B, 1, H, W, 3)
         live._normal_map = out[n3:2 * n3].view(B, 1, H, W, 3)
diff --git a/include/gradslam_hip.h b/include/gradslam_hip.h
--- a/include/gradslam_hip.h
+++ b/include/gradslam_hip.h
@@ -63,6 +63,10 @@
 GS_API int gs_knn1_grid_f32(const float* src, int64_t n_src, const float* tgt, int64_t n_tgt,
                             int64_t* out_idx, float* out_d2, void* scratch, int64_t* unresolved_out_host,
                             void* stream);
+GS_API int gs_knn1_grid_retained_f32(const float* src, int64_t n_src, const float* tgt, int64_t n_tgt,
+                                     int64_t* out_idx, float* out_d2, void* scratch, int scratch_retained,
+                                     int64_t* unresolved_out_host, void* stream);
+GS_API int gs_knn1_grid_counts_range(int64_t n_src, int64_t n_tgt, int64_t* offset_bytes_host, int64_t* n_words_host);
 
 GS_API int gs_gauss_newton_rows_f32(const float* src, int64_t n_src, const float* tgt,
                              const float* tgt_normals, int64_t n_tgt, float dist_thresh,
@@ -292,6 +296,9 @@
 GS_API int gs_pointfusion_step_batch_f32(const gs_step_seq* seqs_host, int B, int H, int W, int ds,
                                          const gs_icp_params* params_host, float two_sigma_sq, float dist_th,
                                          float dot_th, int renorm_all, void* stream);
+GS_API int gs_pointfusion_step_batch_retained_f32(const gs_step_seq* seqs_host, int B, int H, int W, int ds,
+                                                  const gs_icp_params* params_host, float two_sigma_sq, float dist_th,
+                                                  float dot_th, int renorm_all, int scratch_retained, void* stream);
 
 GS_API int gs_project_points_f32(const float* cam_coords, int cdim, int64_t n, const float* proj16, int64_t pts_per_mat,
                                  float* out_uv, void* stream);
```

Result: slower. 2128 (-45.1%).
